# VITA-Group/mm-hand

Hardware: AMD Instinct MI355X
Metric: 256x256 hand images/sec (G+D step) (higher is better)
Workload: dtype f32; 1 GPU; RHD-shaped 256x256, per-GPU batch 32, fp32 (Winograd F(6x6,3x3) on the 3x3 stack), G(9 PATBlocks, ngf64)+D_PB+D_PP+L1/perceptual/GAN+Adam, --norm instance, dropout on; VGG19[:4] weights: random-init (seed 1234): NOT the reference's pretrained objective; global_batch=32, parallelism=dp1

## Files before the change

include/mmhand_hip.h:

```cpp
#ifndef MMHAND_HIP_H
#define MMHAND_HIP_H

#include <stddef.h>
#include <stdint.h>

#ifdef __cplusplus
extern "C" {
#endif
#pragma GCC visibility push(default)

typedef void* mmh_stream_t;

enum { MMH_PAD_ZERO = 0, MMH_PAD_REFLECT = 1 };
enum { MMH_ACT_NONE = 0, MMH_ACT_RELU = 1, MMH_ACT_TANH = 2 };
enum { MMH_F32 = 0, MMH_BF16 = 1, MMH_FP16 = 2 };

typedef struct mmh_conv_desc {
    int32_t B, H, W;
    int32_t Cin, Cout;
    int32_t kh, kw;
    int32_t stride;
    int32_t pad;
    int32_t pad_mode;
    int32_t Ho, Wo;
// ... 150 lines not shown
size_t mmh_colsum_ws_bytes(int64_t rows, int C);
int mmh_colsum(const void* x, int64_t rows, int C, int cs, void* out,
               void* ws, size_t ws_bytes, int accumulate, int x_dtype, mmh_stream_t s);


size_t mmh_norm_stats_ws_bytes(int groups, int64_t rows_per_group, int C);
int mmh_norm_stats(const void* x, int groups, int64_t rows_per_group, int C,
                   int cs, void* mean, void* m2, void* ws, size_t ws_bytes,
                   int x_dtype, mmh_stream_t s);

int mmh_norm_stats_merge(const void* partials, int groups, int chunks, int C, void* mean,
                         void* m2, mmh_stream_t s);

size_t mmh_norm_stats_merge2_ws_bytes(int sub, int C);
int mmh_norm_stats_merge2(const void* partials, int chunks, int C, int sub, void* ws,
                          size_t ws_bytes, void* mean, void* m2, mmh_stream_t s);

int mmh_norm_stats_merge_finalize(const void* partials, int groups, int chunks, int C, double count,
                                  float eps, void* mean, void* m2, void* scale, void* shift,
                                  void* invstd, mmh_stream_t s);
int mmh_syncbn_merge_finalize(const void* gathered, int ranks, int64_t rank_stride, int C, double count,
                              float eps, const void* gamma, const void* beta, void* mean, void* m2,
                              void* scale, void* shift, void* invstd, void* running_mean,
                              void* running_var, float momentum, mmh_stream_t s);
int mmh_norm_finalize(const void* mean, const void* m2, double count,
                      const void* gamma, const void* beta, float eps,
                      int groups, int C, void* scale, void* shift,
                      void* invstd, void* running_mean, void* running_var,
                      float momentum, mmh_stream_t s);

int mmh_scale_shift_act(const void* x, const void* scale, const void* shift,
                        const void* residual, void* out, int groups,
                        int64_t rows_per_group, int C, int relu, float drop_p,
                        uint64_t seed, const void* mask, void* keep_bits,
                        int x_dtype, int out_dtype, mmh_stream_t s);
int mmh_scale_shift_act_twin(const void* x, const void* scale, const void* shift,
                             const void* residual, void* out, int groups,
                             int64_t rows_per_group, int C, int relu, float drop_p,
                             uint64_t seed, const void* mask, void* keep_bits,
                             int x_dtype, int out_dtype, void* twin, int twin_dtype, mmh_stream_t s);

size_t mmh_norm_bwd_ws_bytes(int groups, int64_t rows_per_group, int C);
int mmh_norm_bwd_reduce(const void* g, const void* out, const void* x,
                        const void* mean, const void* invstd, int groups,
                        int64_t rows_per_group, int C, int masked,
                        float drop_p, void* s1, void* s2, void* ws,
                        size_t ws_bytes, int g_dtype, int x_dtype, mmh_stream_t s);
int mmh_norm_bwd_apply(const void* g, const void* out, const void* x,
                       const void* mean, const void* invstd,
                       const void* gamma, const void* s1, const void* s2,
                       double count, int groups, int64_t rows_per_group,
                       int C, int masked, float drop_p, void* dx,
                       int g_dtype, int x_dtype, int dx_dtype, mmh_stream_t s);

int mmh_norm_bwd_fused_supported(int groups, int64_t rows, int C, int masked, int g_dtype, int x_dtype);
int mmh_norm_bwd_fused(const void* g, const void* out, const void* x, const void* mean, const void* invstd,
                       const void* gamma, double count, int groups, int64_t rows, int C, int masked, float drop_p,
                       void* s1, void* s2, void* dx, int g_dtype, int x_dtype, int dx_dtype, mmh_stream_t s);

int mmh_dropout_bits(int64_t n, float drop_p, uint64_t seed, const void* mask, void* bits,
                     mmh_stream_t s);
int mmh_dropout_bits_rows(const void* bits, int64_t image_rows, int W, int C, void* rows,
                          mmh_stream_t s);
int mmh_dropout_bits_both(int64_t image_rows, int W, int C, float drop_p, uint64_t seed,
                          const void* mask, void* bits, void* rows, mmh_stream_t s);
int mmh_norm_bwd_reduce_rc(const void* g, const void* x, const void* mean, const void* invstd,
                           const void* scale, const void* shift, const void* dbits, int groups,
                           int64_t rows_per_group, int C, int relu, float drop_p, void* s1,
                           void* s2, void* ws, size_t ws_bytes, mmh_stream_t s);
int mmh_norm_bwd_apply_rc(const void* g, const void* x, const void* mean, const void* invstd,
                          const void* gamma, const void* s1, const void* s2, const void* scale,
                          const void* shift, const void* dbits, double count, int groups,
                          int64_t rows_per_group, int C, int relu, float drop_p, void* dx,
                          mmh_stream_t s);
int mmh_wino_input_normact(const void* x, int B, int H, int W, int C, int reflect, void* V,
                           const void* scale, const void* shift, int groups, int relu,
                           float drop_p, const void* drows, mmh_stream_t s);
int mmh_wino_input_dy_normbwd(const void* g, const void* x, int B, int H, int W, int C, void* V,
                              void* Yh, int fold, const void* mean, const void* invstd,
                              const void* gamma, const void* s1, const void* s2, double count,
                              const void* scale, const void* shift, const void* drows, int groups,
                              int relu, float drop_p, mmh_stream_t s);

int mmh_act_bwd(const void* g, const void* y, void* dx, int64_t n, int act,
                mmh_stream_t s);
int mmh_act_bwd_lp16(const void* g, const void* y, int64_t n, int act, int dtype, void* out16,
                     mmh_stream_t s);
int mmh_act_bwd_lp16_io(const void* g, int g_is16, const void* y, int y_is16, int64_t n, int act, int dtype,
                        void* out16, mmh_stream_t s);

int mmh_patblock_gate_fwd(const void* x1, const void* s1, const void* s2,
                          const void* s3, void* out, void* x2n, void* x3n,
                          int64_t rows, int C, int cat_dtype, int s23_dtype, mmh_stream_t s);
int mmh_patblock_gate_bwd(const void* g_out, const void* g_x2n,
                          const void* g_x3n, const void* s1, const void* s2,
                          const void* s3, void* g_x1, void* g_s1, void* g_s2,
                          void* g_s3, int64_t rows, int C, int gcat_dtype, int s23_dtype,
                          int gs23_dtype, mmh_stream_t s);

int mmh_patblock_gate_norm_supported(int groups, int64_t rows_per_group, int C);
int mmh_patblock_gate_norm_fwd(const void* x1, const void* y2, const void* scale, const void* shift,
                               const void* s2, const void* s3, void* out, void* x2n, void* x3n, int groups,
                               int64_t rows_per_group, int C, int y_dtype, int cat_dtype, int s23_dtype,
                               mmh_stream_t s);
int mmh_patblock_gate_norm_bwd(const void* g_out, const void* g_x2n, const void* g_x3n, const void* y2,
                               const void* scale, const void* shift, const void* mean, const void* invstd,
                               const void* s2, const void* s3, void* g_x1, void* g_s1, void* g_s2, void* g_s3,
                               void* sum1, void* sum2, void* ws, size_t ws_bytes, int groups,
                               int64_t rows_per_group, int C, int y_dtype, int gcat_dtype, int s23_dtype,
                               mmh_stream_t s);

size_t mmh_reduce_ws_bytes(int64_t n);
int mmh_bce_logits_fwd(const void* x, int64_t n, float target, float weight,
                       double denom, void* out, void* ws, size_t ws_bytes,
                       mmh_stream_t s);
int mmh_bce_logits_bwd(const void* x, int64_t n, float target, float weight,
                       double denom, const void* gscalar, void* dx,
                       mmh_stream_t s);
int mmh_l1_fwd(const void* a, const void* b, int64_t n, float weight,
               double denom, void* out, void* ws, size_t ws_bytes,
               mmh_stream_t s);
int mmh_l1_bwd(const void* a, const void* b, int64_t n, float weight,
               double denom, const void* gscalar, void* da, mmh_stream_t s);
int mmh_l1_fwd_lp16(const void* a16, const void* b16, int64_t n, float weight,
                    double denom, int dtype, void* out, void* ws, size_t ws_bytes,
                    mmh_stream_t s);
int mmh_l1_relu_bwd_lp16(const void* a16, const void* b16, int64_t n, float weight,
                         double denom, const void* gscalar, int dtype, void* out16,
                         mmh_stream_t s);

int mmh_mse_fwd(const void* a, const void* b, int64_t n, float weight,
                double denom, void* out, void* ws, size_t ws_bytes,
                mmh_stream_t s);
int mmh_mse_bwd(const void* a, const void* b, int64_t n, float weight,
                double denom, const void* gscalar, void* da, mmh_stream_t s);

int mmh_maxpool2x2_fwd(const void* x, int B, int H, int W, int C, void* y, mmh_stream_t s);
int mmh_maxpool2x2_bwd(const void* x, const void* g, int B, int H, int W, int C, void* dx, mmh_stream_t s);

int mmh_conv7_thin_fprop(const mmh_conv_desc* d, const void* x, const void* w,
                         const void* bias, void* y, int act, mmh_stream_t s);
size_t mmh_conv7_thin_dgrad_ws_bytes(const mmh_conv_desc* d);
int mmh_conv7_thin_dgrad(const mmh_conv_desc* d, const void* dy, const void* w,
                         void* dx, void* ws, size_t ws_bytes, int dy_dtype, mmh_stream_t s);
size_t mmh_conv7_thin_wgrad_ws_bytes(const mmh_conv_desc* d);
int mmh_conv7_thin_wgrad(const mmh_conv_desc* d, const void* x, const void* dy, void* dw,
                         void* ws, size_t ws_bytes, int accumulate, mmh_stream_t s);

int mmh_conv7_head_dgrad_lp16_supported(const mmh_conv_desc* d);
size_t mmh_conv7_head_dgrad_lp16_ws_bytes(const mmh_conv_desc* d);
int mmh_conv7_head_dgrad_lp16(const mmh_conv_desc* d, const void* dy, const void* w, void* dx, int dx_is16, void* ws,
                              size_t ws_bytes, const void* zeros, mmh_stream_t s);

int mmh_conv7_n4_lp16_supported(const mmh_conv_desc* d, int mode);
size_t mmh_conv7_n4_lp16_ws_bytes(const mmh_conv_desc* d, int mode);
int mmh_conv7_n4_lp16(const mmh_conv_desc* d, int mode, const void* x16, const void* w,
                      const void* bias, void* y, int act, void* ws, size_t ws_bytes,
                      const void* zeros, mmh_stream_t s);

int mmh_conv7_stem_wgrad_supported(const mmh_conv_desc* d);
size_t mmh_conv7_stem_wgrad_ws_bytes(const mmh_conv_desc* d);
int mmh_conv7_stem_wgrad(const mmh_conv_desc* d, const void* x, const void* dy, void* dw,
                         void* ws, size_t ws_bytes, int accumulate, mmh_stream_t s);

int mmh_adam_step(void* p, const void* g, void* m, void* v, int64_t n,
                  float lr, float beta1, float beta2, float eps, int step,
// ... 98 lines not shown
```

mmhand_amd/csrc/common.h:

```cpp
#pragma once
#include <hip/hip_runtime.h>
#include <cstdarg>
#include <cstdio>
#include <cstdint>
#include "../../include/mmhand_hip.h"

namespace mmh {

char* err_buf();
int fail(const char* fmt, ...);

inline int check_launch(const char* what) {
    hipError_t e = hipGetLastError();
    if (e != hipSuccess) return fail("%s: %s", what, hipGetErrorString(e));
    return 0;
}

inline hipStream_t as_stream(mmh_stream_t s) { return reinterpret_cast<hipStream_t>(s); }

inline int64_t cdiv(int64_t a, int64_t b) { return (a + b - 1) / b; }

__device__ __forceinline__ float norm_bwd_elem(float g, bool keep, float dsc, float xv, float mu, float k0, float k1,
                                               float k2) {
    float dz = keep ? g * dsc : 0.f;
// ... 21 lines not shown
        float lo = even[r], hi = odd[r];
        asm volatile("s_nop 1\n\tv_permlane16_swap_b32 %0, %1\n\ts_nop 1" : "+v"(lo), "+v"(hi));
        v[r] = lo;
        v[4 + r] = hi;
    }
}
template <bool H16>
__device__ __forceinline__ void store8_lp16(char* dst, const float* v) {
    if (H16) {
        typedef _Float16 h8 __attribute__((ext_vector_type(8)));
        h8 o;
#pragma unroll
        for (int e = 0; e < 8; ++e) o[e] = (_Float16)v[e];
        *reinterpret_cast<h8*>(dst) = o;
    } else {
        typedef __bf16 b8 __attribute__((ext_vector_type(8)));
        b8 o;
#pragma unroll
        for (int e = 0; e < 8; ++e) o[e] = (__bf16)v[e];
        *reinterpret_cast<b8*>(dst) = o;
    }
}

#define MMH_SWZ_(val, s) __builtin_bit_cast(float, __builtin_amdgcn_ds_swizzle(__builtin_bit_cast(int, val), 0x1f | ((s) << 10)))
template <int NS, int S>
__device__ __forceinline__ void wave_stats_step(float* m, float* q, int& ns, bool bit, float w) {
    if (ns > 1) {
        const int h = ns / 2;
#pragma unroll
        for (int c = 0; c < NS / 2; ++c) {
            if (c < h) {
                const float km = bit ? m[h + c] : m[c], sm = bit ? m[c] : m[h + c];
                const float kq = bit ? q[h + c] : q[c], sq = bit ? q[c] : q[h + c];
                const float om = MMH_SWZ_(sm, S), oq = MMH_SWZ_(sq, S), dl = om - km;
                q[c] = kq + oq + dl * dl * w;
                m[c] = 0.5f * (km + om);
            }
        }
        ns = h;
    } else {
        const float om = MMH_SWZ_(m[0], S), oq = MMH_SWZ_(q[0], S), dl = om - m[0];
        q[0] = q[0] + oq + dl * dl * w;
        m[0] = 0.5f * (m[0] + om);
    }
}
template <int NV, int NJ, typename F>
__device__ __forceinline__ void wave_tile_stats(F val, int l15, float* sp, int N) {
    constexpr int NS = 4 * NJ;
    float m[NS], q[NS];
#pragma unroll
    for (int j = 0; j < NJ; ++j)
#pragma unroll
        for (int r = 0; r < 4; ++r) {
            float v[NV], mean = 0.f, qq = 0.f;
#pragma unroll
            for (int i = 0; i < NV; ++i) { v[i] = val(i, j, r); mean += v[i]; }
            mean *= 1.f / NV;
#pragma unroll
            for (int i = 0; i < NV; ++i) qq = __builtin_fmaf(v[i] - mean, v[i] - mean, qq);
            m[4 * j + r] = mean; q[4 * j + r] = qq;
        }
    int ns = NS;
    wave_stats_step<NS, 8>(m, q, ns, (l15 & 8) != 0, 0.5f * NV);
    wave_stats_step<NS, 4>(m, q, ns, (l15 & 4) != 0, 1.0f * NV);
    wave_stats_step<NS, 2>(m, q, ns, (l15 & 2) != 0, 2.0f * NV);
    wave_stats_step<NS, 1>(m, q, ns, (l15 & 1) != 0, 4.0f * NV);
    constexpr int SPLITS = NS >= 16 ? 4 : (NS >= 8 ? 3 : (NS >= 4 ? 2 : 1));
    const int slot = l15 >> (4 - SPLITS);
    const bool writer = (l15 & ((1 << (4 - SPLITS)) - 1)) == 0;
    if (writer) {
        const int co = (slot >> 2) * 16 + (slot & 3);
        sp[co] = 16.f * NV;
        sp[N + co] = m[0];
        sp[2 * N + co] = q[0];
    }
}

int wino6_weights(const float* w, float* U, int Cin, int Cout, int flip_transpose, hipStream_t st);
int wino6_weights_multi(const long long* table, int n, long long total_blocks, hipStream_t st);
int wino6_input(const float* x, float* V, int B, int H, int W, int C, int reflect, int xcd, hipStream_t st);
int wino6_output(const float* M, float* y, const float* bias, int B, int H, int W, int C, int act, float* stats,
                 int fold, hipStream_t st);
int wino6_dy(const float* dy, float* Yh, int B, int H, int W, int C, hipStream_t st);
int wino6_input_normact(const float* x, float* V, int B, int H, int W, int C, int reflect, int xcd,
                        const float* scale, const float* shift, int groups, int relu, float drop_p,
                        const uint32_t* drows, hipStream_t st);
int wino6_input_dy_normbwd(const float* g, const float* x, float* V, float* Yh, int B, int H, int W, int C, int xcd,
                           int fold, const float* mean, const float* invstd, const float* gamma, const float* s1,
                           const float* s2, double count, const float* scale, const float* shift,
                           const uint32_t* drows, int groups, int relu, float drop_p, hipStream_t st);
int wino6_input_dy(const float* dy, float* V, float* Yh, int B, int H, int W, int C, int xcd, int fold,
                   hipStream_t st);
int wino6_dw(const float* dU, float* dw, int Cin, int Cout, int accumulate, hipStream_t st);
bool wgrad_lp16t_supported(const mmh_conv_desc* d);
int wgrad_lp16t_splits(const mmh_conv_desc* d);
int launch_wgrad_lp16t(const mmh_conv_desc* d, const void* x16, const void* dy16, float* slab, const void* zeros,
                       hipStream_t st);
bool dgrad_s2_halo_ok(const mmh_conv_desc* d, int dx_cs, int act);
int launch_dgrad_s2_halo(const mmh_conv_desc* d, const void* dy, const void* w, const void* bias, void* dx, int dx_cs,
                         int act, hipStream_t st);
extern int g_dgrad_s2_halo, g_dgrad_s2_dbg;
bool wgrad_s2_strip_ok(const mmh_conv_desc* d);
size_t wgrad_s2_strip_ws_bytes(const mmh_conv_desc* d);
int launch_wgrad_s2_strip(const mmh_conv_desc* d, const void* x, const void* dy, void* dw, void* ws, size_t ws_bytes,
                          int accumulate, hipStream_t st);
extern int g_wgrad_s2_strip;
bool stem_f32_ok(const mmh_conv_desc* d);
int stem_f32_stats_chunks(const mmh_conv_desc* d);
int launch_stem_f32(const mmh_conv_desc* d, const void* x, const void* w, const void* bias, void* y, int act, float* stats,
                    hipStream_t st);
extern int g_stem_f32, g_stem_f32_dbg, g_stem_f32_levels;
bool wino_wgrad_dma_ok(int64_t tiles, int Cin, int Cout, int nbatch);
size_t wino_wgrad_dma_ws_bytes(int64_t tiles, int Cin, int Cout, int nbatch);
int launch_wino_wgrad_dma(const float* V, const float* Yh, int64_t tiles, int Cin, int Cout, int nbatch, float* ws, float* dU,
                          hipStream_t st);
extern int g_wino_wgrad_dma;
int launch_slab_reduce(const float* slab, float* dw, int64_t n4_total, int splits, int accumulate, int64_t n4, hipStream_t st);
bool conv_s2f_ok(const mmh_conv_desc* d, int mode);
bool conv_s1f_ok(const mmh_conv_desc* d, int mode);
int conv_s2f_stats_chunks(const mmh_conv_desc* d);
int launch_conv_s2f(const mmh_conv_desc* d, const void* x16, const void* w16, const void* bias, void* y, int y_is16, int act,
                    const void* zeros, hipStream_t st, float* stats = nullptr, int mode = 0);
bool conv_s2d_ok(const mmh_conv_desc* d, int mode);
int launch_conv_s2d(const mmh_conv_desc* d, const void* g16, const void* w16, const void* bias, void* dx, int dx_is16, int act,
                    const void* zeros, hipStream_t st);
extern int g_lp16_s2f;
extern int g_lp16_persist;
extern int g_slab_reduce_par;
extern int g_wino6_vec;
extern int g_lp16_shape;
extern int g_lp16_tap_inner;
extern int g_lp16_dbg;
extern int g_lp16_wgrad_ring;
extern int g_lp16_wgrad_s2;
extern int g_pw_v2;
extern int g_col_chunks, g_row_chunks;

}

#define MMH_REQUIRE(cond, ...)                      \
    do {                                            \
        if (!(cond)) return mmh::fail(__VA_ARGS__); \
    } while (0)
```

mmhand_amd/csrc/conv_igemm.hip:

```cpp
#include <algorithm>
#include <cstring>
#include "common.h"

namespace {

typedef float f32x16 __attribute__((ext_vector_type(16)));
typedef __bf16 bf16x8 __attribute__((ext_vector_type(8)));
typedef __bf16 bf16x4 __attribute__((ext_vector_type(4)));
typedef __bf16 bf16x2 __attribute__((ext_vector_type(2)));
typedef _Float16 f16x8 __attribute__((ext_vector_type(8)));
typedef _Float16 f16x4 __attribute__((ext_vector_type(4)));
typedef _Float16 f16x2 __attribute__((ext_vector_type(2)));
__device__ __forceinline__ bf16x4 to_bf16x4(float4 v) {
    bf16x4 r;
    r[0] = (__bf16)v.x; r[1] = (__bf16)v.y; r[2] = (__bf16)v.z; r[3] = (__bf16)v.w;
    return r;
}
template <bool H16>
__device__ __forceinline__ bf16x4 to_lp4(float4 v) {
    if (H16) {
        f16x4 r;
        r[0] = (_Float16)v.x; r[1] = (_Float16)v.y; r[2] = (_Float16)v.z; r[3] = (_Float16)v.w;
        return __builtin_bit_cast(bf16x4, r);
    }
// ... 2638 lines not shown
            v.x = apply_act(v.x, act); v.y = apply_act(v.y, act);
            yo[(((long long)b * H + 4 * ty + r) * W + 4 * tx + q) * C2 + c] = v;
        }
    }
}

__global__ void wino4_dy_kernel(const float* __restrict__ dy, float* __restrict__ Yh, int B, int H, int W,
                                int C2) {
    const int TH = H / 4, TW = W / 4;
    const long long tiles = (long long)B * TH * TW;
    long long i = (long long)blockIdx.x * blockDim.x + threadIdx.x;
    if (i >= tiles * C2) return;
    const int c = (int)(i % C2);
    const long long tile = i / C2;
    const int tx = (int)(tile % TW), ty = (int)((tile / TW) % TH), b = (int)(tile / ((long long)TW * TH));
    const F2* in = reinterpret_cast<const F2*>(dy);
    F2 yv[4][4], t[6][4], colv[4], o6[6];
#pragma unroll
    for (int r = 0; r < 4; ++r)
#pragma unroll
        for (int q = 0; q < 4; ++q) yv[r][q] = in[(((long long)b * H + 4 * ty + r) * W + 4 * tx + q) * C2 + c];
#pragma unroll
    for (int q = 0; q < 4; ++q) {
#pragma unroll
        for (int r = 0; r < 4; ++r) colv[r] = yv[r][q];
        w4_a(colv, o6);
#pragma unroll
        for (int r = 0; r < 6; ++r) t[r][q] = o6[r];
    }
    const long long plane = tiles * C2;
    F2* out = reinterpret_cast<F2*>(Yh) + tile * C2 + c;
#pragma unroll
    for (int r = 0; r < 6; ++r) {
        w4_a(t[r], o6);
#pragma unroll
        for (int q = 0; q < 6; ++q) out[(long long)(r * 6 + q) * plane] = o6[q];
    }
}

__global__ void wino4_dw_kernel(const float* __restrict__ dU, float* __restrict__ dw, int64_t plane2,
                                int accumulate) {
    int64_t i = (int64_t)blockIdx.x * blockDim.x + threadIdx.x;
    if (i >= plane2) return;
    const F2* in = reinterpret_cast<const F2*>(dU) + i;
    F2 u[6][6], t[3][6], colv[6], o3[3];
#pragma unroll
    for (int a = 0; a < 6; ++a)
#pragma unroll
        for (int b = 0; b < 6; ++b) u[a][b] = in[(int64_t)(a * 6 + b) * plane2];
#pragma unroll
    for (int b = 0; b < 6; ++b) {
#pragma unroll
        for (int a = 0; a < 6; ++a) colv[a] = u[a][b];
        w4_gt(colv, o3);
#pragma unroll
        for (int a = 0; a < 3; ++a) t[a][b] = o3[a];
    }
    F2* out = reinterpret_cast<F2*>(dw) + i;
#pragma unroll
    for (int a = 0; a < 3; ++a) {
        w4_gt(t[a], o3);
#pragma unroll
        for (int b = 0; b < 3; ++b) {
            F2 v = o3[b];
            if (accumulate) v = v + out[(int64_t)(a * 3 + b) * plane2];
            out[(int64_t)(a * 3 + b) * plane2] = v;
        }
    }
}

template <int BN, int WM, int WN, bool NMAJOR>
int launch_batched_t(const BatchKP& bp, int nbatch, hipStream_t st) {
    constexpr size_t lds = (BM * LDA + (NMAJOR ? BN * LDA : BK * BN)) * sizeof(float) + tab_bytes(BM);
    static int ready = -1;
    if (ready != 0) ready = allow_lds(conv_igemm_batched_kernel<BN, WM, WN, NMAJOR>, lds);
    if (ready != 0) return ready;
    dim3 grid((bp.p.N + BN - 1) / BN, (bp.p.M + BM - 1) / BM, nbatch);
    hipLaunchKernelGGL((conv_igemm_batched_kernel<BN, WM, WN, NMAJOR>), grid, dim3(256), lds, st, bp);
    return mmh::check_launch("conv_igemm_batched_kernel");
}

int g_wino_bn256 = 0;
int g_wino_xcd = 1;
int g_wino_gemm_v2 = 1;
int g_wino_bf16_bk = 64;
int g_wino_bf16_occ = 3;
int g_wino_gemm_occ = 3;
int g_wino_gemm_levels = 2;
int g_wino_gemm_bn = 0;

template <int BN, int LEVELS>
static int launch_wino_gemm_t(const WinoGemmKP& p, hipStream_t st) {
    constexpr size_t lds = (size_t)(BM * LDA + BK * BN) * sizeof(float);
    static int ready = -1;
    if (ready != 0) ready = allow_lds(wino_gemm_kernel<BN, LEVELS>, lds);
    if (ready != 0) return ready;
    hipLaunchKernelGGL((wino_gemm_kernel<BN, LEVELS>), dim3(8 * p.nb), dim3(256), lds, st, p);
    return mmh::check_launch("wino_gemm_kernel");
}

static int wino_gemm_v2(const float* V, const float* U, float* Mo, long long tiles, int K, int N, hipStream_t st,
                        int nbatch, int levels, bool fold16 = false) {
    WinoGemmKP p{};
    p.A = V; p.B = U; p.C = Mo;
    p.M = (int)tiles; p.K = K; p.N = N; p.P = nbatch;
    const int bn = g_wino_gemm_bn == 64 ? 64 : (N > 64 ? 128 : 64);
    p.MT = (p.M + BM - 1) / BM;
    p.NT = (N + bn - 1) / bn;
    p.W = nbatch * p.MT * p.NT;
    p.Wx = (p.W + 7) / 8;
    const bool two = (levels ? levels : g_wino_gemm_levels) == 2 && (nbatch == 64 || fold16) && K > WINO_FOLD * BK;
    p.nb = std::min(p.Wx, 32 * g_wino_gemm_occ);
    if (two) return bn == 128 ? launch_wino_gemm_t<128, 2>(p, st) : launch_wino_gemm_t<64, 2>(p, st);
    return bn == 128 ? launch_wino_gemm_t<128, 1>(p, st) : launch_wino_gemm_t<64, 1>(p, st);
}

int wino_gemm(const float* V, const float* U, float* Mo, long long tiles, int K, int N, hipStream_t st,
              int nbatch = 16, int levels = 0) {
    MMH_REQUIRE(tiles * (long long)std::max(K, N) < (1ll << 30), "winograd: tensor too large");
    if (g_wino_gemm_v2 && K % BK == 0 && N >= 64 && N % 32 == 0) return wino_gemm_v2(V, U, Mo, tiles, K, N, st, nbatch, levels);
    BatchKP bp{};
    ConvKP& p = bp.p;
    Gather& g = p.g;
    g.src = V;
    g.src_bytes = (unsigned)((size_t)tiles * K * sizeof(float));
    g.srcH = 1; g.srcW = (int)tiles; g.src_cs = (unsigned)K;
    g.PH = 1; g.PW = (int)tiles; g.TH = 1; g.TW = 1;
    g.C4 = K / 4;
    g.ap_h = 0; g.at_h = 0; g.a0_h = 0; g.ap_w = 1; g.at_w = 0; g.a0_w = 0;
    g.shift = 0; g.reflect = 0;
    set_korder(g, p.nk, p.Kflat);
    p.w = U;
    p.w_bytes = (unsigned)((size_t)K * N * sizeof(float));
    p.out = Mo;
    p.M = (int)tiles; p.N = N;
    p.wCin = K; p.wCout = N;
    p.KW_true = 1; p.kh0 = 0; p.kw0 = 0; p.tstep = 1;
    p.OH = 1; p.OW = (int)tiles; p.o_p = 1;
    p.out_cs = (unsigned)N; p.out_linear = 1;
    p.act = MMH_ACT_NONE;
    bp.src_bs = tiles * K; bp.w_bs = (long long)K * N; bp.out_bs = tiles * N;
    {
        const int bn = (N % 256 == 0 && g_wino_bn256) ? 256 : 128;
        const int gx = (N + bn - 1) / bn, gy = (p.M + BM - 1) / BM;
        p.xcd_remap = (g_conv_xcd && gx > 1 && gy >= 8) ? 1 : 0;
    }
    if (N % 256 == 0 && g_wino_bn256) return launch_batched_t<256, 2, 2, false>(bp, nbatch, st);
    if (N > 64) return launch_batched_t<128, 2, 2, false>(bp, nbatch, st);
    if (N > 32) return launch_batched_t<64, 2, 2, false>(bp, nbatch, st);
    return launch_batched_t<32, 4, 1, false>(bp, nbatch, st);
}

int g_wgrad_slots = 768;
int g_wgrad_bn256 = 1;
int g_wino_wgrad_v2 = 1;
int g_wino_wgrad_occ = 3;
int g_wgrad_xcd = 1;
int g_wino_wgrad_bn256 = 0;
int g_wino_wgrad_slots = 2304;

int wgrad_splits(int Mrows, int N, int P) {
    const int bn = (g_wgrad_bn256 && N % 256 == 0) ? 256 : 128;
    const int tiles = ((Mrows + BM - 1) / BM) * ((N + bn - 1) / bn);
    const int slots = g_wgrad_slots;
    int max_splits = P / (8 * BK);
    if (max_splits > 256) max_splits = 256;
// ... 43 lines not shown

template <int BN, int WM, int WN>
int launch_wgrad_grid_t(const WgradKP& p, dim3 grid, hipStream_t st) {
    constexpr size_t lds = (BK * LDW + BK * BN) * sizeof(float);
    static int ready = -1;
    if (ready != 0) ready = allow_lds(conv_wgrad_kernel<BN, WM, WN, false>, lds);
    if (ready != 0) return ready;
    hipLaunchKernelGGL((conv_wgrad_kernel<BN, WM, WN, false>), grid, dim3(256), lds, st, p);
    return mmh::check_launch("conv_wgrad_kernel");
}

size_t wgrad_ws(const mmh_conv_desc* d) {
    const int Mrows = d->kh * d->kw * d->Cin;
    const int P = d->B * d->Ho * d->Wo;
    const size_t generic = (size_t)wgrad_splits(Mrows, d->Cout, P) * Mrows * d->Cout * sizeof(float);
    return mmh::wgrad_s2_strip_ok(d) ? std::max(generic, mmh::wgrad_s2_strip_ws_bytes(d)) : generic;
}

int do_wgrad(const mmh_conv_desc* d, const void* x, const void* dy, void* dw, void* ws,
             size_t ws_bytes, int accumulate, hipStream_t st, bool x16 = false, bool dy16 = false) {
    MMH_REQUIRE(!(x16 || dy16) || is16(d->dtype), "wgrad: 16-bit operands need a 16-bit dtype");
    MMH_REQUIRE(x16 == dy16, "wgrad: io16 must be 0 (both tensors fp32) or 3 (both 16-bit)");
    if (!x16 && mmh::wgrad_s2_strip_ok(d)) return mmh::launch_wgrad_s2_strip(d, x, dy, dw, ws, ws_bytes, accumulate, st);
    WgradKP p{};
    p.g = fwd_gather(d, x);
    p.g.chunk_major = 0;
    p.x16 = x16 ? 1 : 0;
    p.dy16 = dy16 ? 1 : 0;
    if (x16) p.g.src_bytes /= 2;
    p.dy = static_cast<const float*>(dy);
    p.dy_bytes = (unsigned)((size_t)d->B * d->Ho * d->Wo * d->y_cs * (dy16 ? 2 : sizeof(float)));
    p.dy_cs = (unsigned)d->y_cs;
    p.Mrows = d->kh * d->kw * d->Cin;
    p.N = d->Cout;
    p.P = d->B * d->Ho * d->Wo;
    const int splits = wgrad_splits(p.Mrows, p.N, p.P);
    MMH_REQUIRE(ws_bytes >= (size_t)splits * p.Mrows * p.N * sizeof(float),
                "wgrad workspace too small: %zu < %zu", ws_bytes,
                (size_t)splits * p.Mrows * p.N * sizeof(float));
    p.slab = static_cast<float*>(ws);
    const bool bf16 = is16(d->dtype);
    p.h16 = d->dtype == MMH_FP16;
    p.pix_per_split = (int)(mmh::cdiv(mmh::cdiv(p.P, splits), bf16 ? BKP : BK) * (bf16 ? BKP : BK));
    p.dbg = g_conv_dbg;
    p.nsplit = splits;
    int rc;
    if (bf16) {
        if (p.N > 64) rc = launch_wgrad_bf16_t<128, 2, 2>(p, splits, st);
        else if (p.N > 32) rc = launch_wgrad_bf16_t<64, 2, 2>(p, splits, st);
        else rc = launch_wgrad_bf16_t<32, 4, 1>(p, splits, st);
    } else if (g_wgrad_bn256 && p.N % 256 == 0) rc = launch_wgrad_t<256, 2, 2, false>(p, splits, st);
    else if (p.N > 64) rc = g_wgrad_dbuf ? launch_wgrad_t<128, 2, 2, true>(p, splits, st)
                                    : launch_wgrad_t<128, 2, 2, false>(p, splits, st);
    else if (p.N > 32) rc = launch_wgrad_t<64, 2, 2, false>(p, splits, st);
    else rc = launch_wgrad_t<32, 4, 1, false>(p, splits, st);
    if (rc) return rc;
    const int64_t n4 = (int64_t)p.Mrows * p.N / 4;
    return mmh::launch_slab_reduce(p.slab, static_cast<float*>(dw), n4, splits, accumulate, n4, st);
}

}

extern "C" {

int mmh_set_option(const char* key, int value) {
    MMH_REQUIRE(key != nullptr, "mmh_set_option: NULL key");
    if (!strcmp(key, "conv_dbuf")) { g_conv_dbuf = value; return 0; }
    if (!strcmp(key, "conv_dbg")) { g_conv_dbg = value; return 0; }
    if (!strcmp(key, "conv_cw")) { g_conv_cw = value; return 0; }
    if (!strcmp(key, "conv_bn256")) { g_conv_bn256 = value; return 0; }
    if (!strcmp(key, "conv_levels")) { g_conv_levels = value == 2 ? 2 : 1; mmh::g_stem_f32_levels = g_conv_levels; return 0; }
    if (!strcmp(key, "wino_bn256")) { g_wino_bn256 = value; return 0; }
    if (!strcmp(key, "conv_xcd")) { g_conv_xcd = value; return 0; }
    if (!strcmp(key, "conv_xcd1")) { g_conv_xcd1 = value; return 0; }
    if (!strcmp(key, "conv_tall")) { g_conv_tall = value; return 0; }
    if (!strcmp(key, "wgrad_slots")) { g_wgrad_slots = value; return 0; }
    if (!strcmp(key, "wgrad_dbuf")) { g_wgrad_dbuf = value; return 0; }
    if (!strcmp(key, "wgrad_bn256")) { g_wgrad_bn256 = value; return 0; }
    if (!strcmp(key, "wgrad_xcd")) { g_wgrad_xcd = value; return 0; }
    if (!strcmp(key, "wino_wgrad_v2")) { g_wino_wgrad_v2 = value; return 0; }
    if (!strcmp(key, "wino_wgrad_occ")) { g_wino_wgrad_occ = value; return 0; }
    if (!strcmp(key, "wino_gemm_v2")) { g_wino_gemm_v2 = value; return 0; }
    if (!strcmp(key, "wino_xcd")) { g_wino_xcd = value; return 0; }
    if (!strcmp(key, "dgrad_s2_multi")) { g_dgrad_s2_multi = value; return 0; }
    if (!strcmp(key, "wino6_vec")) { mmh::g_wino6_vec = value; return 0; }
    if (!strcmp(key, "lp16_shape")) { mmh::g_lp16_shape = value; return 0; }
    if (!strcmp(key, "lp16_s2f")) { mmh::g_lp16_s2f = value; return 0; }
    if (!strcmp(key, "lp16_persist")) { mmh::g_lp16_persist = value; return 0; }
    if (!strcmp(key, "lp16_tap_inner")) { mmh::g_lp16_tap_inner = value; return 0; }
    if (!strcmp(key, "pw_v2")) { mmh::g_pw_v2 = value; return 0; }
    if (!strcmp(key, "col_chunks") && value > 0) { mmh::g_col_chunks = value; return 0; }
    if (!strcmp(key, "row_chunks") && value > 0) { mmh::g_row_chunks = value; return 0; }
    if (!strcmp(key, "dgrad_s2_halo")) { mmh::g_dgrad_s2_halo = value; return 0; }
    if (!strcmp(key, "wgrad_s2_strip")) { mmh::g_wgrad_s2_strip = value; return 0; }
    if (!strcmp(key, "stem_f32")) { mmh::g_stem_f32 = value; return 0; }
    if (!strcmp(key, "wino_wgrad_dma")) { mmh::g_wino_wgrad_dma = value; return 0; }
    if (!strcmp(key, "stem_f32_dbg")) { mmh::g_stem_f32_dbg = value; return 0; }
    if (!strcmp(key, "slab_reduce_par")) { mmh::g_slab_reduce_par = value; return 0; }
    if (!strcmp(key, "dgrad_s2_dbg")) { mmh::g_dgrad_s2_dbg = value; return 0; }
    if (!strcmp(key, "lp16_dbg")) { mmh::g_lp16_dbg = value; return 0; }
    if (!strcmp(key, "lp16_wgrad_ring")) { mmh::g_lp16_wgrad_ring = value; return 0; }
    if (!strcmp(key, "lp16_wgrad_s2")) { mmh::g_lp16_wgrad_s2 = value; return 0; }
    if (!strcmp(key, "border_bn64")) { g_border_bn64 = value; return 0; }
    if (!strcmp(key, "wino_gemm_occ")) { g_wino_gemm_occ = value; return 0; }
    if (!strcmp(key, "wino_gemm_levels")) { g_wino_gemm_levels = value; return 0; }
    if (!strcmp(key, "wino_gemm_bn")) { g_wino_gemm_bn = value; return 0; }
    if (!strcmp(key, "wino_bf16_occ")) { g_wino_bf16_occ = value; return 0; }
    if (!strcmp(key, "wino_bf16_bk")) { g_wino_bf16_bk = value; return 0; }
    if (!strcmp(key, "wino_wgrad_bn256")) { g_wino_wgrad_bn256 = value; return 0; }
    if (!strcmp(key, "wino_wgrad_slots")) { g_wino_wgrad_slots = value; return 0; }
    return mmh::fail("mmh_set_option: unknown key '%s'", key);
}

int mmh_conv2d_fprop(const mmh_conv_desc* d, const void* x, const void* w, const void* bias,
                     void* y, int act, mmh_stream_t s) {
    if (int rc = validate(d)) return rc;
    MMH_REQUIRE(x && w && y, "mmh_conv2d_fprop: NULL buffer");
    return do_fprop(d, x, w, bias, y, act, mmh::as_stream(s));
}

int mmh_conv2d_fprop_stats_chunks(const mmh_conv_desc* d) { return d ? fprop_stats_chunks(d) : 0; }

int mmh_conv2d_fprop_stats(const mmh_conv_desc* d, const void* x, const void* w, const void* bias, void* y,
                           void* stats, mmh_stream_t s) {
    if (int rc = validate(d)) return rc;
    MMH_REQUIRE(x && w && y && stats, "mmh_conv2d_fprop_stats: NULL buffer");
    MMH_REQUIRE(fprop_stats_chunks(d) > 0, "mmh_conv2d_fprop_stats: needs fp32 and B*Ho*Wo %% 128 == 0");
    return do_fprop(d, x, w, bias, y, MMH_ACT_NONE, mmh::as_stream(s), static_cast<float*>(stats));
}

int mmh_conv2d_dgrad(const mmh_conv_desc* d, const void* dy, const void* w, void* dx, int dx_cs,
                     mmh_stream_t s) {
    if (int rc = validate(d)) return rc;
    MMH_REQUIRE(dy && w && dx, "mmh_conv2d_dgrad: NULL buffer");
    MMH_REQUIRE(dx_cs % 4 == 0 && dx_cs >= d->Cin, "mmh_conv2d_dgrad: bad dx_cs=%d", dx_cs);
    return do_dgrad(d, dy, w, nullptr, dx, dx_cs, MMH_ACT_NONE, mmh::as_stream(s));
}

static int wino_planes(int tile) { return (tile + 2) * (tile + 2); }
static bool wino_tile_ok(int tile) { return tile == 2 || tile == 4 || tile == 6; }
static bool wino_hw_ok(int H, int W, int tile) {
    return tile == 6 ? (H >= 4 && W >= 4) : (H >= tile + 2 && W >= tile + 2 && H % tile == 0 && W % tile == 0);
}
static long long wino_tiles(int B, int H, int W, int tile) {
    return (long long)B * ((H + tile - 1) / tile) * ((W + tile - 1) / tile);
}

static bool wino_dtype_ok(int dtype, int tile) { return dtype == MMH_F32 || (is16(dtype) && tile == 2); }

int mmh_wino_weights(const void* w, int Cin, int Cout, int flip_transpose, int tile, int dtype, void* U,
                     mmh_stream_t s) {
    MMH_REQUIRE(w && U && Cin > 0 && Cout > 0 && wino_tile_ok(tile) && wino_dtype_ok(dtype, tile),
                "mmh_wino_weights: bad arguments (tile 2 | 4 | 6; bf16 needs tile 2)");
    const dim3 grid((Cin * Cout + 255) / 256);
    if (tile == 6)
        return mmh::wino6_weights(static_cast<const float*>(w), static_cast<float*>(U), Cin, Cout, flip_transpose,
                                  mmh::as_stream(s));
    if (tile == 4)
        hipLaunchKernelGGL(wino4_weights_kernel, grid, dim3(256), 0, mmh::as_stream(s),
                           static_cast<const float*>(w), static_cast<float*>(U), Cin, Cout, flip_transpose);
    else if (dtype == MMH_FP16)
        hipLaunchKernelGGL(wino_weights_kernel<2>, grid, dim3(256), 0, mmh::as_stream(s),
                           static_cast<const float*>(w), U, Cin, Cout, flip_transpose);
    else if (dtype == MMH_BF16)
        hipLaunchKernelGGL(wino_weights_kernel<1>, grid, dim3(256), 0, mmh::as_stream(s),
                           static_cast<const float*>(w), U, Cin, Cout, flip_transpose);
// ... 122 lines not shown
    p.h16 = h16;
    p.MT = (p.M + BM - 1) / BM;
    p.NT = (N + 127) / 128;
    p.W = nbatch * p.MT * p.NT;
    p.Wx = (p.W + 7) / 8;
    if (g_wino_bf16_bk == 128 && K % 128 == 0) {
        p.nb = std::min(p.Wx, 32 * 2);
        constexpr size_t lds = (size_t)(2 * BM * (128 + 8)) * sizeof(__bf16);
        static int ready = -1;
        if (ready != 0) ready = allow_lds(wino_gemm_bf16_kernel<128, false>, lds) | allow_lds(wino_gemm_bf16_kernel<128, true>, lds);
        if (ready != 0) return ready;
        if (h16) hipLaunchKernelGGL((wino_gemm_bf16_kernel<128, true>), dim3(8 * p.nb), dim3(256), lds, st, p);
        else hipLaunchKernelGGL((wino_gemm_bf16_kernel<128, false>), dim3(8 * p.nb), dim3(256), lds, st, p);
    } else {
        p.nb = std::min(p.Wx, 32 * g_wino_bf16_occ);
        constexpr size_t lds = (size_t)(2 * BM * (64 + 8)) * sizeof(__bf16);
        static int ready = -1;
        if (ready != 0) ready = allow_lds(wino_gemm_bf16_kernel<64, false>, lds) | allow_lds(wino_gemm_bf16_kernel<64, true>, lds);
        if (ready != 0) return ready;
        if (h16) hipLaunchKernelGGL((wino_gemm_bf16_kernel<64, true>), dim3(8 * p.nb), dim3(256), lds, st, p);
        else hipLaunchKernelGGL((wino_gemm_bf16_kernel<64, false>), dim3(8 * p.nb), dim3(256), lds, st, p);
    }
    return mmh::check_launch("wino_gemm_bf16_kernel");
}

int mmh_wino_gemm(const void* V, const void* U, void* M, int64_t tiles, int K, int N, int nbatch, int dtype,
                  mmh_stream_t s) {
    MMH_REQUIRE(V && U && M && tiles > 0 && K % 32 == 0 && N % 4 == 0 && nbatch > 0 &&
                    (dtype == MMH_F32 || is16(dtype)),
                "mmh_wino_gemm: bad arguments");
    if (is16(dtype)) return wino_gemm_bf16(V, U, M, tiles, K, N, nbatch, dtype == MMH_FP16, mmh::as_stream(s));
    return wino_gemm(static_cast<const float*>(V), static_cast<const float*>(U), static_cast<float*>(M), tiles,
                     K, N, mmh::as_stream(s), nbatch);
}

int mmh_wino_gemm_levels(const void* V, const void* U, void* M, int64_t tiles, int K, int N, int nbatch, int levels,
                         mmh_stream_t s) {
    MMH_REQUIRE(V && U && M && tiles > 0 && K % 32 == 0 && N % 4 == 0 && nbatch > 0 && (levels == 1 || levels == 2),
                "mmh_wino_gemm_levels: bad arguments (fp32; levels 1 | 2)");
    return wino_gemm(static_cast<const float*>(V), static_cast<const float*>(U), static_cast<float*>(M), tiles, K, N,
                     mmh::as_stream(s), nbatch, levels);
}

int mmh_wino_gemm_levels16(const void* V, const void* U, void* M, int64_t tiles, int K, int N, int levels, mmh_stream_t s) {
    MMH_REQUIRE(V && U && M && tiles > 0 && K > 0 && K % 32 == 0 && N >= 64 && N % 32 == 0 && (levels == 1 || levels == 2),
                "mmh_wino_gemm_levels16: bad arguments (fp32, 16 planes; K %% 32 == 0, N %% 32 == 0, N >= 64; levels 1 | 2)");
    MMH_REQUIRE(tiles * (long long)std::max(K, N) < (1ll << 30), "mmh_wino_gemm_levels16: tensor too large");
    MMH_REQUIRE(g_wino_gemm_v2, "mmh_wino_gemm_levels16: needs the persistent kernel (option wino_gemm_v2)");
    return wino_gemm_v2(static_cast<const float*>(V), static_cast<const float*>(U), static_cast<float*>(M), tiles, K, N,
                        mmh::as_stream(s), 16, levels, true);
}

int mmh_wino_output(const void* M, void* y, const void* bias, int B, int H, int W, int C, int act, int tile,
                    int dtype, void* stats, int fold, mmh_stream_t s) {
    MMH_REQUIRE(M && y && B > 0 && wino_tile_ok(tile) && wino_hw_ok(H, W, tile) && C % 4 == 0 &&
                    wino_dtype_ok(dtype, tile),
                "mmh_wino_output: bad arguments");
    const long long tiles = wino_tiles(B, H, W, tile);
    MMH_REQUIRE(!stats || (tile == 6 && dtype == MMH_F32), "mmh_wino_output: statistics need tile 6, fp32");
    MMH_REQUIRE(!fold || (tile == 6 && dtype == MMH_F32 && wino_fold_ok(H, W) && !bias && !stats && act == MMH_ACT_NONE),
                "mmh_wino_output: fold needs tile 6, fp32, no bias / activation / statistics, (H+1) %% 6 >= 2");
    if (tile == 6)
        return mmh::wino6_output(static_cast<const float*>(M), static_cast<float*>(y), static_cast<const float*>(bias),
                                 B, H, W, C, act, static_cast<float*>(stats), fold ? 1 : 0, mmh::as_stream(s));
    if (tile == 4) {
        const long long total = tiles * (C / 2);
        hipLaunchKernelGGL(wino4_output_kernel, dim3((unsigned)((total + 255) / 256)), dim3(256), 0,
                           mmh::as_stream(s), static_cast<const float*>(M), static_cast<float*>(y),
                           static_cast<const float*>(bias), B, H, W, C / 2, act);
    } else {
        const long long total = tiles * (C / 4);
        const dim3 grid((unsigned)((total + 255) / 256));
        if (dtype == MMH_FP16)
            hipLaunchKernelGGL(wino_output_kernel<2>, grid, dim3(256), 0, mmh::as_stream(s), M,
                               static_cast<float*>(y), static_cast<const float*>(bias), B, H, W, C / 4, act);
        else if (dtype == MMH_BF16)
            hipLaunchKernelGGL(wino_output_kernel<1>, grid, dim3(256), 0, mmh::as_stream(s), M,
                               static_cast<float*>(y), static_cast<const float*>(bias), B, H, W, C / 4, act);
        else
            hipLaunchKernelGGL(wino_output_kernel<0>, grid, dim3(256), 0, mmh::as_stream(s), M,
                               static_cast<float*>(y), static_cast<const float*>(bias), B, H, W, C / 4, act);
    }
    return mmh::check_launch("wino_output_kernel");
}

static int wino_wgrad_splits(int Cin, int Cout, long long tiles, int nbatch) {
    const int bn = (g_wino_wgrad_bn256 && Cout % 256 == 0) ? 256 : 128;
    const int per = ((Cin + BM - 1) / BM) * ((Cout + bn - 1) / bn) * nbatch;
    const int s = std::max(1, g_wino_wgrad_slots / per);
    const long long maxs = std::max<long long>(1, tiles / (8 * BK));
    return (int)std::min<long long>(s, maxs);
}

size_t mmh_wino_wgrad_gemm_ws_bytes(int64_t tiles, int Cin, int Cout, int nbatch) {
    if (tiles <= 0 || Cin <= 0 || Cout <= 0 || nbatch <= 0) return 0;
    const size_t generic = (size_t)nbatch * wino_wgrad_splits(Cin, Cout, tiles, nbatch) * Cin * Cout * sizeof(float);
    return mmh::wino_wgrad_dma_ok(tiles, Cin, Cout, nbatch) ? std::max(generic, mmh::wino_wgrad_dma_ws_bytes(tiles, Cin, Cout, nbatch))
                                                            : generic;
}

int mmh_wino_wgrad_gemm(const void* V, const void* Yh, int64_t tiles, int Cin, int Cout, int nbatch, int dtype,
                        void* ws, size_t ws_bytes, void* dU, mmh_stream_t s) {
    MMH_REQUIRE(V && Yh && ws && dU && tiles > 0 && Cin % 4 == 0 && Cout % 4 == 0 &&
                    (dtype == MMH_F32 || is16(dtype)),
                "mmh_wino_wgrad_gemm: bad arguments");
    MMH_REQUIRE(ws_bytes >= mmh_wino_wgrad_gemm_ws_bytes(tiles, Cin, Cout, nbatch),
                "mmh_wino_wgrad_gemm: workspace too small");
    MMH_REQUIRE(tiles * (long long)std::max(Cin, Cout) < (1ll << 30), "mmh_wino_wgrad_gemm: tensor too large");
    hipStream_t st = mmh::as_stream(s);
    if (dtype == MMH_F32 && mmh::wino_wgrad_dma_ok(tiles, Cin, Cout, nbatch))
        return mmh::launch_wino_wgrad_dma(static_cast<const float*>(V), static_cast<const float*>(Yh), tiles, Cin, Cout, nbatch,
                                          static_cast<float*>(ws), static_cast<float*>(dU), st);
    const int splits = wino_wgrad_splits(Cin, Cout, tiles, nbatch);
    if (is16(dtype)) {
        MMH_REQUIRE(Cin % BM == 0 && Cout % 128 == 0, "mmh_wino_wgrad_gemm (bf16): needs Cin, Cout %% 128 == 0");
        WinoWgradBfKP q{};
        q.h16 = dtype == MMH_FP16;
        q.V = static_cast<const __bf16*>(V); q.Y = static_cast<const __bf16*>(Yh); q.slab = static_cast<float*>(ws);
        q.T = (int)tiles; q.Cin = Cin; q.Cout = Cout; q.P = nbatch;
        q.t_per_split = (int)(mmh::cdiv(mmh::cdiv(tiles, splits), BKP) * BKP);
        q.S = (int)mmh::cdiv(tiles, q.t_per_split);
        q.MT = Cin / BM; q.NT = Cout / 128;
        q.W = nbatch * q.S * q.MT * q.NT;
        q.Wx = (q.W + 7) / 8;
        q.nb = std::min(q.Wx, 32 * g_wino_bf16_occ);
        constexpr size_t lds = (size_t)(2 * BKP * LDT) * sizeof(__bf16);
        static int ready = -1;
        if (ready != 0) ready = allow_lds(wino_wgrad_gemm_bf16_kernel<false>, lds) | allow_lds(wino_wgrad_gemm_bf16_kernel<true>, lds);
        if (ready != 0) return ready;
        if (q.h16) hipLaunchKernelGGL(wino_wgrad_gemm_bf16_kernel<true>, dim3(8 * q.nb), dim3(256), lds, st, q);
        else hipLaunchKernelGGL(wino_wgrad_gemm_bf16_kernel<false>, dim3(8 * q.nb), dim3(256), lds, st, q);
        if (int rc = mmh::check_launch("wino_wgrad_gemm_bf16_kernel")) return rc;
        const int64_t n4 = (int64_t)Cin * Cout / 4;
        return mmh::launch_slab_reduce(q.slab, static_cast<float*>(dU), nbatch * n4, q.S, 0, n4, st);
    }
    if (g_wino_wgrad_v2 && Cin % BM == 0 && Cout % 128 == 0) {
        WinoWgradKP q{};
        q.V = static_cast<const float*>(V); q.Y = static_cast<const float*>(Yh); q.slab = static_cast<float*>(ws);
        q.T = (int)tiles; q.Cin = Cin; q.Cout = Cout; q.P = nbatch;
        q.t_per_split = (int)(mmh::cdiv(mmh::cdiv(tiles, splits), BK) * BK);
        q.S = (int)mmh::cdiv(tiles, q.t_per_split);
        q.MT = Cin / BM; q.NT = Cout / 128;
        q.W = nbatch * q.S * q.MT * q.NT;
        q.Wx = (q.W + 7) / 8;
        const int occ = g_wino_wgrad_occ == 4 ? 4 : 3;
        q.nb = std::min(q.Wx, 32 * occ);
        constexpr size_t lds = (size_t)(BK * LDW + BK * 128) * sizeof(float);
        static int ready3 = -1, ready4 = -1;
        if (occ == 4) {
            if (ready4 != 0) ready4 = allow_lds(wino_wgrad_gemm_kernel<4>, lds);
            if (ready4 != 0) return ready4;
            hipLaunchKernelGGL(wino_wgrad_gemm_kernel<4>, dim3(8 * q.nb), dim3(256), lds, st, q);
        } else {
            if (ready3 != 0) ready3 = allow_lds(wino_wgrad_gemm_kernel<3>, lds);
            if (ready3 != 0) return ready3;
            hipLaunchKernelGGL(wino_wgrad_gemm_kernel<3>, dim3(8 * q.nb), dim3(256), lds, st, q);
        }
        if (int rc = mmh::check_launch("wino_wgrad_gemm_kernel")) return rc;
        const int64_t n4 = (int64_t)Cin * Cout / 4;
        return mmh::launch_slab_reduce(q.slab, static_cast<float*>(dU), nbatch * n4, q.S, 0, n4, st);
    }
    WgradKP p{};
    Gather& g = p.g;
    g.src = static_cast<const float*>(V);
    g.src_bytes = (unsigned)((size_t)tiles * Cin * sizeof(float));
    g.srcH = 1; g.srcW = (int)tiles; g.src_cs = (unsigned)Cin;
// ... 126 lines not shown
```

mmhand_amd/csrc/wino6.hip:

```cpp
#include "common.h"

namespace {

struct F2 { float x, y; };
__device__ __forceinline__ F2 operator+(F2 a, F2 b) { return {a.x + b.x, a.y + b.y}; }
__device__ __forceinline__ F2 operator-(F2 a, F2 b) { return {a.x - b.x, a.y - b.y}; }
__device__ __forceinline__ F2 operator*(float k, F2 a) { return {k * a.x, k * a.y}; }

__device__ __forceinline__ float act6(float v, int act) {
    if (act == MMH_ACT_RELU) return v > 0.f ? v : 0.f;
    if (act == MMH_ACT_TANH) return tanhf(v);
    return v;
}

template <typename T>
__device__ __forceinline__ void w6_bt(const T* d, T* o) {
    const T e1 = d[2] - 4.25f * d[4] + d[6], f1 = d[1] - 4.25f * d[3] + d[5];
    const T e2 = 0.25f * d[2] - 1.25f * d[4] + d[6], f2 = 0.5f * d[1] - 2.5f * d[3] + 2.f * d[5];
    const T e3 = 4.f * d[2] - 5.f * d[4] + d[6], f3 = 2.f * d[1] - 2.5f * d[3] + 0.5f * d[5];
    o[0] = d[0] - d[6] + 5.25f * (d[4] - d[2]);
    o[1] = e1 + f1; o[2] = e1 - f1;
    o[3] = e2 + f2; o[4] = e2 - f2;
    o[5] = e3 + f3; o[6] = e3 - f3;
    o[7] = d[7] - d[1] + 5.25f * (d[3] - d[5]);
// ... 262 lines not shown
    const long long tiles = (long long)B * TH * TW;
    const long long i = (long long)blockIdx.x * blockDim.x + threadIdx.x;
    if (i >= tiles * C2) return;
    const int c = (int)(i % C2);
    const long long tile = i / C2;
    const int tx = (int)(tile % TW), ty = (int)((tile / TW) % TH), b = (int)(tile / ((long long)TW * TH));
    const long long plane = tiles * C2;
    const T* in = reinterpret_cast<const T*>(M) + tile * C2 + c;
    T s6[6][8], colv[8], o6[6];
#pragma unroll
    for (int q = 0; q < 8; ++q) {
#pragma unroll
        for (int r = 0; r < 8; ++r) colv[r] = in[(long long)(r * 8 + q) * plane];
        w6_at(colv, o6);
#pragma unroll
        for (int r = 0; r < 6; ++r) s6[r][q] = o6[r];
    }
    const T bv = bias ? reinterpret_cast<const T*>(bias)[c] : zero_of(T{});
    T* yo = reinterpret_cast<T*>(y);
    T vals[6][6];
    if (fold) {
#pragma unroll
        for (int r = 0; r < 6; ++r) {
            w6_at(s6[r], o6);
#pragma unroll
            for (int q = 0; q < 6; ++q) vals[r][q] = o6[q];
        }
        const int rb = H + 1 - 6 * ty, cb = W + 1 - 6 * tx;
#pragma unroll
        for (int q = 0; q < 6; ++q) {
            if (ty == 0) vals[2][q] = vals[2][q] + vals[0][q];
#pragma unroll
            for (int r = 2; r < 6; ++r)
                if (r == rb) vals[r - 2][q] = vals[r - 2][q] + vals[r][q];
        }
#pragma unroll
        for (int r = 0; r < 6; ++r) {
            if (tx == 0) vals[r][2] = vals[r][2] + vals[r][0];
#pragma unroll
            for (int q = 2; q < 6; ++q)
                if (q == cb) vals[r][q - 2] = vals[r][q - 2] + vals[r][q];
        }
#pragma unroll
        for (int r = 0; r < 6; ++r) {
            const int ph = 6 * ty + r;
#pragma unroll
            for (int q = 0; q < 6; ++q) {
                const int pw = 6 * tx + q;
                if (ph >= 1 && ph <= H && pw >= 1 && pw <= W)
                    yo[(((long long)b * H + ph - 1) * W + pw - 1) * C2 + c] = vals[r][q];
            }
        }
        return;
    }
    float n = 0.f, sum = 0.f;
#pragma unroll
    for (int r = 0; r < 6; ++r) {
        const int hh = 6 * ty + r;
        w6_at(s6[r], o6);
#pragma unroll
        for (int q = 0; q < 6; ++q) {
            const int ww = 6 * tx + q;
            vals[r][q] = act_of(o6[q] + bv, act);
            if (hh < H && ww < W) {
                yo[(((long long)b * H + hh) * W + ww) * C2 + c] = vals[r][q];
                stat_add(vals[r][q], n, sum);
            }
        }
    }
    if (stats && sizeof(T) == 4) {
        const float mean = sum / n;
        float m2 = 0.f;
#pragma unroll
        for (int r = 0; r < 6; ++r)
#pragma unroll
            for (int q = 0; q < 6; ++q)
                if (6 * ty + r < H && 6 * tx + q < W) {
                    const float d = *reinterpret_cast<const float*>(&vals[r][q]) - mean;
                    m2 += d * d;
                }
        float* o = stats + ((long long)(b * (TH * TW) + ty * TW + tx) * 3) * C2 + c;
        o[0] = n; o[C2] = mean; o[2 * C2] = m2;
    }
}

template <typename T>
__global__ void __launch_bounds__(256) wino6_dy_kernel(const float* __restrict__ dy, float* __restrict__ Yh, int B,
                                                       int H, int W, int C2) {
    const int TH = (H + 5) / 6, TW = (W + 5) / 6;
    const long long tiles = (long long)B * TH * TW;
    const long long i = (long long)blockIdx.x * blockDim.x + threadIdx.x;
    if (i >= tiles * C2) return;
    const int c = (int)(i % C2);
    const long long tile = i / C2;
    const int tx = (int)(tile % TW), ty = (int)((tile / TW) % TH), b = (int)(tile / ((long long)TW * TH));
    const T* in = reinterpret_cast<const T*>(dy);
    T t[8][6], colv[6], o8[8];
#pragma unroll
    for (int q = 0; q < 6; ++q) {
        const int ww = 6 * tx + q;
#pragma unroll
        for (int r = 0; r < 6; ++r) {
            const int hh = 6 * ty + r;
            colv[r] = (hh < H && ww < W) ? in[(((long long)b * H + hh) * W + ww) * C2 + c] : zero_of(T{});
        }
        w6_a(colv, o8);
#pragma unroll
        for (int r = 0; r < 8; ++r) t[r][q] = o8[r];
    }
    const long long plane = tiles * C2;
    T* out = reinterpret_cast<T*>(Yh) + tile * C2 + c;
#pragma unroll
    for (int r = 0; r < 8; ++r) {
        w6_a(t[r], o8);
#pragma unroll
        for (int q = 0; q < 8; ++q) out[(long long)(r * 8 + q) * plane] = o8[q];
    }
}

template <typename T>
__device__ __forceinline__ void dy_transforms(T (&d)[8][8], float* __restrict__ V, float* __restrict__ Yh,
                                              long long plane, long long at, int fold) {
    T colv[8], o8[8];
    {
        T t[8][6];
#pragma unroll
        for (int q = 0; q < 6; ++q) {
#pragma unroll
            for (int r = 0; r < 6; ++r) colv[r] = fold ? d[r + 2][q + 2] : d[r + 1][q + 1];
            w6_a(colv, o8);
#pragma unroll
            for (int r = 0; r < 8; ++r) t[r][q] = o8[r];
        }
        T* out = reinterpret_cast<T*>(Yh) + at;
#pragma unroll
        for (int r = 0; r < 8; ++r) {
            w6_a(t[r], o8);
#pragma unroll
            for (int q = 0; q < 8; ++q) out[(long long)(r * 8 + q) * plane] = o8[q];
        }
    }
#pragma unroll
    for (int q = 0; q < 8; ++q) {
#pragma unroll
        for (int r = 0; r < 8; ++r) colv[r] = d[r][q];
        w6_bt(colv, o8);
#pragma unroll
        for (int r = 0; r < 8; ++r) d[r][q] = o8[r];
    }
    T* out = reinterpret_cast<T*>(V) + at;
#pragma unroll
    for (int r = 0; r < 8; ++r) {
        w6_bt(d[r], o8);
#pragma unroll
        for (int q = 0; q < 8; ++q) out[(long long)(r * 8 + q) * plane] = o8[q];
    }
}

template <typename T>
__global__ void __launch_bounds__(256) wino6_input_dy_kernel(const float* __restrict__ dy, float* __restrict__ V,
                                                             float* __restrict__ Yh, int B, int H, int W, int C2,
                                                             int xcd_remap, int fold) {
    const int org = fold ? 2 : 1;
    const int TH = (H + 5) / 6, TW = (W + 5) / 6;
    const long long tiles = (long long)B * TH * TW;
    unsigned blk = blockIdx.x;
// ... 87 lines not shown
                const int rr = 2 * stage + r;
                bool keep = !nb.relu || __builtin_fmaf(xw[r][q], sc, sf) > 0.f;
                if (DROP) {
                    const uint32_t wsel = (wg.ww[q] >> 5) == wq0 ? lo[r] : hi[r];
                    keep = keep && ((wsel >> (wg.ww[q] & 31)) & 1u);
                }
                const float o = mmh::norm_bwd_elem(d[rr][q], keep, nb.np.dsc, xw[r][q], mu, k0, k1, k2);
                d[rr][q] = (wg.okh[rr] && wg.okw[q]) ? o : 0.f;
            }
        __builtin_amdgcn_sched_barrier(0);
    }
    dy_transforms(d, V, Yh, tiles * C, tile * C + c, fold);
}

__global__ void __launch_bounds__(256) wino6_dw_kernel(const float* __restrict__ dU, float* __restrict__ dw, int64_t plane2, int accumulate) {
    const int64_t i = (int64_t)blockIdx.x * blockDim.x + threadIdx.x;
    if (i >= plane2) return;
    const F2* in = reinterpret_cast<const F2*>(dU) + i;
    F2 t[3][8], colv[8], o3[3];
#pragma unroll
    for (int q = 0; q < 8; ++q) {
#pragma unroll
        for (int r = 0; r < 8; ++r) colv[r] = in[(int64_t)(r * 8 + q) * plane2];
        w6_gt(colv, o3);
#pragma unroll
        for (int r = 0; r < 3; ++r) t[r][q] = o3[r];
    }
    F2* out = reinterpret_cast<F2*>(dw) + i;
#pragma unroll
    for (int a = 0; a < 3; ++a) {
        w6_gt(t[a], o3);
#pragma unroll
        for (int b = 0; b < 3; ++b) {
            F2 v = o3[b];
            if (accumulate) v = v + out[(int64_t)(a * 3 + b) * plane2];
            out[(int64_t)(a * 3 + b) * plane2] = v;
        }
    }
}

}

namespace mmh {

int wino6_weights(const float* w, float* U, int Cin, int Cout, int flip_transpose, hipStream_t st) {
    hipLaunchKernelGGL(wino6_weights_kernel, dim3((Cin * Cout + 255) / 256), dim3(256), 0, st, w, U, Cin, Cout,
                       flip_transpose);
    return check_launch("wino6_weights_kernel");
}

int wino6_weights_multi(const long long* table, int n, long long total_blocks, hipStream_t st) {
    hipLaunchKernelGGL(wino6_weights_multi_kernel, dim3((unsigned)total_blocks), dim3(256), 0, st, table, n);
    return check_launch("wino6_weights_multi_kernel");
}

int g_wino6_vec = 0x0;

int wino6_input(const float* x, float* V, int B, int H, int W, int C, int reflect, int xcd, hipStream_t st) {
    const int ext = reflect == 2 ? 7 : 5;
    const long long tiles = (long long)B * ((H + ext) / 6) * ((W + ext) / 6);
    const int cpt = (g_wino6_vec & 1) ? 2 : 1;
    const unsigned nblk = (unsigned)((tiles * (C / cpt) + 255) / 256);
    const int remap = (xcd && nblk % 8 == 0 && nblk >= 64) ? 1 : 0;
    if (cpt == 2)
        hipLaunchKernelGGL(wino6_input_kernel<F2>, dim3(nblk), dim3(256), 0, st, x, V, B, H, W, C / 2, reflect, remap);
    else
        hipLaunchKernelGGL(wino6_input_kernel<float>, dim3(nblk), dim3(256), 0, st, x, V, B, H, W, C, reflect, remap);
    return check_launch("wino6_input_kernel");
}

int wino6_output(const float* M, float* y, const float* bias, int B, int H, int W, int C, int act, float* stats,
                 int fold, hipStream_t st) {
    const int ext = fold ? 7 : 5;
    const long long tiles = (long long)B * ((H + ext) / 6) * ((W + ext) / 6);
    if ((g_wino6_vec & 2) && !stats)
        hipLaunchKernelGGL(wino6_output_kernel<F2>, dim3((unsigned)((tiles * (C / 2) + 255) / 256)), dim3(256), 0, st, M,
                           y, bias, B, H, W, C / 2, act, nullptr, fold);
    else
        hipLaunchKernelGGL(wino6_output_kernel<float>, dim3((unsigned)((tiles * C + 255) / 256)), dim3(256), 0, st, M, y,
                           bias, B, H, W, C, act, stats, fold);
    return check_launch("wino6_output_kernel");
}

int wino6_dy(const float* dy, float* Yh, int B, int H, int W, int C, hipStream_t st) {
    const long long tiles = (long long)B * ((H + 5) / 6) * ((W + 5) / 6);
    if (g_wino6_vec & 4)
        hipLaunchKernelGGL(wino6_dy_kernel<F2>, dim3((unsigned)((tiles * (C / 2) + 255) / 256)), dim3(256), 0, st, dy, Yh,
                           B, H, W, C / 2);
    else
        hipLaunchKernelGGL(wino6_dy_kernel<float>, dim3((unsigned)((tiles * C + 255) / 256)), dim3(256), 0, st, dy, Yh, B,
                           H, W, C);
    return check_launch("wino6_dy_kernel");
}

int wino6_input_normact(const float* x, float* V, int B, int H, int W, int C, int reflect, int xcd,
                        const float* scale, const float* shift, int groups, int relu, float drop_p,
                        const uint32_t* drows, hipStream_t st) {
    const long long tiles = (long long)B * ((H + 5) / 6) * ((W + 5) / 6);
    const unsigned nblk = (unsigned)((tiles * C + 255) / 256);
    const int remap = (xcd && nblk % 8 == 0 && nblk >= 64) ? 1 : 0;
    NormPro np{scale, shift, drows, (W + 31) / 32, groups == 1 ? 0 : 1, relu ? 0.f : -INFINITY, 1.f / (1.f - drop_p)};
    if (drows)
        hipLaunchKernelGGL(wino6_input_normact_kernel<true>, dim3(nblk), dim3(256), 0, st, x, V, B, H, W, C, reflect,
                           remap, np);
    else
        hipLaunchKernelGGL(wino6_input_normact_kernel<false>, dim3(nblk), dim3(256), 0, st, x, V, B, H, W, C, reflect,
                           remap, np);
    return check_launch("wino6_input_normact_kernel");
}

int wino6_input_dy_normbwd(const float* g, const float* x, float* V, float* Yh, int B, int H, int W, int C, int xcd,
                           int fold, const float* mean, const float* invstd, const float* gamma, const float* s1,
                           const float* s2, double count, const float* scale, const float* shift,
                           const uint32_t* drows, int groups, int relu, float drop_p, hipStream_t st) {
    const long long tiles = (long long)B * ((H + 5) / 6) * ((W + 5) / 6);
    const unsigned nblk = (unsigned)((tiles * C + 255) / 256);
    const int remap = (xcd && nblk % 8 == 0 && nblk >= 64) ? 1 : 0;
    NormBwdPro nb{x, mean, invstd, gamma, s1, s2, (float)(1.0 / count), relu,
                  NormPro{scale, shift, drows, (W + 31) / 32, groups == 1 ? 0 : 1, 0.f, 1.f / (1.f - drop_p)}};
    if (drows)
        hipLaunchKernelGGL(wino6_input_dy_normbwd_kernel<true>, dim3(nblk), dim3(256), 0, st, g, V, Yh, B, H, W, C, remap,
                           fold, nb);
    else
        hipLaunchKernelGGL(wino6_input_dy_normbwd_kernel<false>, dim3(nblk), dim3(256), 0, st, g, V, Yh, B, H, W, C, remap,
                           fold, nb);
    return check_launch("wino6_input_dy_normbwd_kernel");
}

int wino6_input_dy(const float* dy, float* V, float* Yh, int B, int H, int W, int C, int xcd, int fold,
                   hipStream_t st) {
    const long long tiles = (long long)B * ((H + 5) / 6) * ((W + 5) / 6);
    const unsigned nblk = (unsigned)((tiles * C + 255) / 256);
    hipLaunchKernelGGL(wino6_input_dy_kernel<float>, dim3(nblk), dim3(256), 0, st, dy, V, Yh, B, H, W, C,
                       (xcd && nblk % 8 == 0 && nblk >= 64) ? 1 : 0, fold);
    return check_launch("wino6_input_dy_kernel");
}

int wino6_dw(const float* dU, float* dw, int Cin, int Cout, int accumulate, hipStream_t st) {
    const int64_t n2 = (int64_t)Cin * Cout / 2;
    hipLaunchKernelGGL(wino6_dw_kernel, dim3((unsigned)cdiv(n2, 256)), dim3(256), 0, st, dU, dw, n2, accumulate);
    return check_launch("wino6_dw_kernel");
}

}
```

mmhand_amd/lib.py:

```python
import ctypes as C
import os

_HERE = os.path.dirname(os.path.abspath(__file__))
LIB_PATH = os.environ.get("MMH_LIB_PATH") or os.path.join(_HERE, "libmmhand_hip.so")

PAD_ZERO, PAD_REFLECT = 0, 1
ACT_NONE, ACT_RELU, ACT_TANH = 0, 1, 2
F32, BF16, FP16 = 0, 1, 2
U8 = 3


class ConvDesc(C.Structure):
    _fields_ = [(n, C.c_int32) for n in (
        "B", "H", "W", "Cin", "Cout", "kh", "kw", "stride", "pad", "pad_mode",
        "Ho", "Wo", "x_cs", "y_cs", "dtype")]


class PlaneSrc(C.Structure):
    _fields_ = [("ptr", C.c_void_p), ("C", C.c_int32),
                ("sb", C.c_int64), ("sc", C.c_int64), ("sh", C.c_int64), ("sw", C.c_int64)]


class ImageSrc(C.Structure):
    _fields_ = [("ptr", C.c_void_p), ("dtype", C.c_int32), ("scale", C.c_float), ("offset", C.c_float),
# ... 42 lines not shown
    "mmh_conv7_thin_dgrad_ws_bytes": (_sz, [_DP]),
    "mmh_conv7_thin_dgrad": (_i, [_DP, _vp, _vp, _vp, _vp, _sz, _i, _vp]),
    "mmh_conv7_thin_wgrad_ws_bytes": (_sz, [_DP]),
    "mmh_conv7_thin_wgrad": (_i, [_DP, _vp, _vp, _vp, _vp, _sz, _i, _vp]),
    "mmh_conv7_stem_wgrad_supported": (_i, [_DP]),
    "mmh_conv7_stem_wgrad_ws_bytes": (_sz, [_DP]),
    "mmh_conv7_stem_wgrad": (_i, [_DP, _vp, _vp, _vp, _vp, _sz, _i, _vp]),
    "mmh_conv2d_wgrad_ws_bytes": (_sz, [_DP]),
    "mmh_conv2d_wgrad": (_i, [_DP, _vp, _vp, _vp, _vp, _sz, _i, _i, _vp]),
    "mmh_convT2d_fprop": (_i, [_DP, _vp, _vp, _vp, _vp, _i, _i, _vp]),
    "mmh_convT2d_dgrad": (_i, [_DP, _vp, _vp, _vp, _vp]),
    "mmh_convT2d_wgrad": (_i, [_DP, _vp, _vp, _vp, _vp, _sz, _i, _i, _vp]),
    "mmh_reflect_fold": (_i, [_vp, _vp, _i, _i, _i, _i, _i, _vp]),
    "mmh_prep_weights_bf16": (_i, [_vp, _i, _i, _i, _vp, _vp, _vp]),
    "mmh_prep_weights_bf16_flat": (_i, [_vp, _i, _i, _i, _vp, _vp]),
    "mmh_prep_weights_fp16": (_i, [_vp, _i, _i, _i, _vp, _vp, _vp]),
    "mmh_prep_weights_fp16_flat": (_i, [_vp, _i, _i, _i, _vp, _vp]),
    "mmh_cvt_lp16": (_i, [_vp, _i64, _i, _vp, _vp]),
    "mmh_conv_lp16_supported": (_i, [_DP, _i]),
    "mmh_conv_lp16": (_i, [_DP, _i, _vp, _vp, _vp, _vp, _i, _i, _vp, _vp]),
    "mmh_conv_lp16_stats_chunks": (_i, [_DP]),
    "mmh_conv_lp16_fprop_stats": (_i, [_DP, _vp, _vp, _vp, _vp, _vp, _vp, _vp]),
    "mmh_conv_stem16_stats_chunks": (_i, [_DP, _i]),
    "mmh_conv_stem16_stats": (_i, [_DP, _vp, _i, _vp, _vp, _vp, _vp, _vp, _vp]),
    "mmh_lp16_pad_cvt": (_i, [_vp, _i64, _i, _i, _i, _vp, _vp]),
    "mmh_prep_weights_lp16_flat8": (_i, [_vp, _i, _i, _i, _i, _i, _vp, _vp]),
    "mmh_conv_lp16_flat_supported": (_i, [_DP, _i]),
    "mmh_conv_lp16_flat": (_i, [_DP, _vp, _i, _vp, _vp, _vp, _i, _i, _vp, _vp]),
    "mmh_conv_stem16_supported": (_i, [_DP, _i]),
    "mmh_dgrad_s2_halo_supported": (_i, [_DP, _i]),
    "mmh_conv_stem16_weights_bytes": (_sz, [_i]),
    "mmh_prep_weights_stem16": (_i, [_vp, _i, _i, _i, _vp, _vp]),
    "mmh_conv_stem16_weights_bytes_k": (_sz, [_i, _i]),
    "mmh_prep_weights_stem16_k": (_i, [_vp, _i, _i, _i, _i, _vp, _vp]),
    "mmh_conv_stem16": (_i, [_DP, _vp, _i, _vp, _vp, _vp, _i, _i, _vp, _vp]),
    "mmh_wgrad_stem_lp16_supported": (_i, [_DP, _i]),
    "mmh_wgrad_stem_lp16_ws_bytes": (_sz, [_DP, _i]),
    "mmh_wgrad_stem_lp16": (_i, [_DP, _vp, _i, _vp, _vp, _vp, _sz, _i, _vp, _vp]),
    "mmh_conv7_head_wgrad_lp16_supported": (_i, [_DP]),
    "mmh_conv7_head_wgrad_lp16_ws_bytes": (_sz, [_DP]),
    "mmh_conv7_head_wgrad_lp16": (_i, [_DP, _vp, _vp, _vp, _vp, _sz, _i, _vp, _vp]),
    "mmh_wgrad_lp16_flat_supported": (_i, [_DP, _i]),
    "mmh_wgrad_lp16_flat_ws_bytes": (_sz, [_DP, _i]),
    "mmh_wgrad_lp16_flat": (_i, [_DP, _vp, _i, _i, _vp, _vp, _vp, _sz, _i, _vp, _vp]),
    "mmh_conv7_head_dgrad_lp16_supported": (_i, [_DP]),
    "mmh_conv7_head_dgrad_lp16_ws_bytes": (_sz, [_DP]),
    "mmh_conv7_head_dgrad_lp16": (_i, [_DP, _vp, _vp, _vp, _i, _vp, _sz, _vp, _vp]),
    "mmh_conv7_n4_lp16_supported": (_i, [_DP, _i]),
    "mmh_conv7_n4_lp16_ws_bytes": (_sz, [_DP, _i]),
    "mmh_conv7_n4_lp16": (_i, [_DP, _i, _vp, _vp, _vp, _vp, _i, _vp, _sz, _vp, _vp]),
    "mmh_conv3x3_lp16_supported": (_i, [_DP]),
    "mmh_conv3x3_lp16_fold_supported": (_i, [_DP]),
    "mmh_wgrad3x3_lp16_ws_bytes": (_sz, [_DP]),
    "mmh_wgrad3x3_lp16": (_i, [_DP, _vp, _vp, _vp, _vp, _sz, _i, _vp, _vp]),
    "mmh_conv3x3_lp16": (_i, [_DP, _i, _vp, _vp, _vp, _vp, _i, _i, _vp, _vp]),
    "mmh_conv3x3_lp16_stats_chunks": (_i, [_DP]),
    "mmh_conv3x3_lp16_dgrad_nbr_chunks": (_i, [_DP, _i]),
    "mmh_conv3x3_lp16_dgrad_nbr": (_i, [_DP, _i, _vp, _vp, _vp, _vp, _vp, _vp, _vp, _i, _f, _vp, _vp, _vp, _sz, _vp, _vp]),
    "mmh_norm_bwd_sums_final": (_i, [_vp, _i, _i, _i, _vp, _vp, _vp]),
    "mmh_conv3x3_lp16_dgrad_add_supported": (_i, [_DP]),
    "mmh_conv3x3_lp16_dgrad_add": (_i, [_DP, _i, _vp, _vp, _vp, _vp, _vp, _vp]),
    "mmh_conv3x3_lp16_fprop_stats": (_i, [_DP, _vp, _vp, _vp, _vp, _vp, _vp, _vp]),
    "mmh_colsum_ws_bytes": (_sz, [_i64, _i]),
    "mmh_colsum": (_i, [_vp, _i64, _i, _i, _vp, _vp, _sz, _i, _i, _vp]),
    "mmh_norm_stats_ws_bytes": (_sz, [_i, _i64, _i]),
    "mmh_norm_stats": (_i, [_vp, _i, _i64, _i, _i, _vp, _vp, _vp, _sz, _i, _vp]),
    "mmh_norm_finalize": (_i, [_vp, _vp, _d, _vp, _vp, _f, _i, _i, _vp, _vp, _vp, _vp, _vp, _f, _vp]),
    "mmh_syncbn_merge_finalize": (_i, [_vp, _i, _i64, _i, _d, _f, _vp, _vp, _vp, _vp, _vp, _vp, _vp, _vp, _vp, _f, _vp]),
    "mmh_scale_shift_act": (_i, [_vp, _vp, _vp, _vp, _vp, _i, _i64, _i, _i, _f, _u64, _vp, _vp, _i, _i, _vp]),
    "mmh_scale_shift_act_twin": (_i, [_vp, _vp, _vp, _vp, _vp, _i, _i64, _i, _i, _f, _u64, _vp, _vp, _i, _i, _vp, _i, _vp]),
    "mmh_norm_bwd_ws_bytes": (_sz, [_i, _i64, _i]),
    "mmh_norm_bwd_reduce": (_i, [_vp, _vp, _vp, _vp, _vp, _i, _i64, _i, _i, _f, _vp, _vp, _vp, _sz, _i, _i, _vp]),
    "mmh_norm_bwd_apply": (_i, [_vp, _vp, _vp, _vp, _vp, _vp, _vp, _vp, _d, _i, _i64, _i, _i, _f, _vp, _i, _i, _i, _vp]),
    "mmh_norm_bwd_fused_supported": (_i, [_i, _i64, _i, _i, _i, _i]),
    "mmh_norm_bwd_fused": (_i, [_vp, _vp, _vp, _vp, _vp, _vp, _d, _i, _i64, _i, _i, _f, _vp, _vp, _vp, _i, _i, _i, _vp]),
    "mmh_dropout_bits": (_i, [_i64, _f, _u64, _vp, _vp, _vp]),
    "mmh_dropout_bits_rows": (_i, [_vp, _i64, _i, _i, _vp, _vp]),
    "mmh_dropout_bits_both": (_i, [_i64, _i, _i, _f, _u64, _vp, _vp, _vp, _vp]),
    "mmh_norm_bwd_reduce_rc": (_i, [_vp, _vp, _vp, _vp, _vp, _vp, _vp, _i, _i64, _i, _i, _f, _vp, _vp, _vp, _sz, _vp]),
    "mmh_norm_bwd_apply_rc": (_i, [_vp, _vp, _vp, _vp, _vp, _vp, _vp, _vp, _vp, _vp, _d, _i, _i64, _i, _i, _f, _vp, _vp]),
    "mmh_wino_input_normact": (_i, [_vp, _i, _i, _i, _i, _i, _vp, _vp, _vp, _i, _i, _f, _vp, _vp]),
    "mmh_wino_input_dy_normbwd": (_i, [_vp, _vp, _i, _i, _i, _i, _vp, _vp, _i, _vp, _vp, _vp, _vp, _vp, _d, _vp, _vp,
                                       _vp, _i, _i, _f, _vp]),
    "mmh_act_bwd": (_i, [_vp, _vp, _vp, _i64, _i, _vp]),
    "mmh_act_bwd_lp16": (_i, [_vp, _vp, _i64, _i, _i, _vp, _vp]),
    "mmh_act_bwd_lp16_io": (_i, [_vp, _i, _vp, _i, _i64, _i, _i, _vp, _vp]),
    "mmh_patblock_gate_fwd": (_i, [_vp, _vp, _vp, _vp, _vp, _vp, _vp, _i64, _i, _i, _i, _vp]),
    "mmh_patblock_gate_bwd": (_i, [_vp, _vp, _vp, _vp, _vp, _vp, _vp, _vp, _vp, _vp, _i64, _i, _i, _i, _i, _vp]),
    "mmh_patblock_gate_norm_supported": (_i, [_i, _i64, _i]),
    "mmh_patblock_gate_norm_fwd": (_i, [_vp, _vp, _vp, _vp, _vp, _vp, _vp, _vp, _vp, _i, _i64, _i, _i, _i, _i, _vp]),
    "mmh_patblock_gate_norm_bwd": (_i, [_vp, _vp, _vp, _vp, _vp, _vp, _vp, _vp, _vp, _vp, _vp, _vp, _vp, _vp, _vp, _vp, _vp, _sz,
                                        _i, _i64, _i, _i, _i, _i, _vp]),
    "mmh_reduce_ws_bytes": (_sz, [_i64]),
    "mmh_bce_logits_fwd": (_i, [_vp, _i64, _f, _f, _d, _vp, _vp, _sz, _vp]),
    "mmh_bce_logits_bwd": (_i, [_vp, _i64, _f, _f, _d, _vp, _vp, _vp]),
    "mmh_l1_fwd": (_i, [_vp, _vp, _i64, _f, _d, _vp, _vp, _sz, _vp]),
    "mmh_l1_bwd": (_i, [_vp, _vp, _i64, _f, _d, _vp, _vp, _vp]),
    "mmh_l1_fwd_lp16": (_i, [_vp, _vp, _i64, _f, _d, _i, _vp, _vp, _sz, _vp]),
    "mmh_l1_relu_bwd_lp16": (_i, [_vp, _vp, _i64, _f, _d, _vp, _i, _vp, _vp]),
    "mmh_mse_fwd": (_i, [_vp, _vp, _i64, _f, _d, _vp, _vp, _sz, _vp]),
    "mmh_maxpool2x2_fwd": (_i, [_vp, _i, _i, _i, _i, _vp, _vp]),
    "mmh_maxpool2x2_bwd": (_i, [_vp, _vp, _i, _i, _i, _i, _vp, _vp]),
    "mmh_mse_bwd": (_i, [_vp, _vp, _i64, _f, _d, _vp, _vp, _vp]),
    "mmh_adam_step": (_i, [_vp, _vp, _vp, _vp, _i64, _f, _f, _f, _f, _i, _f, _vp, _vp, _vp]),
    "mmh_grad_nonfinite": (_i, [_vp, _i64, _vp, _vp, _vp, _vp]),
    "mmh_loss_scale_update": (_i, [_vp, _vp, _f, _f, _i, _f, _f, _vp]),
    "mmh_pack_nhwc": (_i, [C.POINTER(PlaneSrc), _i, _vp, _i, _i, _i, _i, _i, _vp]),
    "mmh_pack_nhwc_lp16": (_i, [C.POINTER(PlaneSrc), _i, _vp, _vp, _i, _i, _i, _i, _i, _i, _vp]),
    "mmh_pose_heatmaps": (_i, [_vp, _i, _i, _i, _d, _vp, _vp]),
    "mmh_map_to_cord": (_i, [_vp, _i, _i, _i, _f, _vp, _vp]),
    "mmh_decode_inputs": (_i, [_vp, _vp, _vp, _vp, _vp, _vp, _i, _i, _i, _d, _vp, _vp, _vp, _vp, _vp]),
    "mmh_decode_inputs_resized": (_i, [_vp, _vp, _vp, _vp, _vp, _vp, _i, _i, _i, _i, _i, _d, _vp, _vp, _vp, _vp, _vp]),
    "mmh_rccl_bind": (_i, [C.c_char_p]),
    "mmh_rccl_comm_ranks": (_i, [_vp]),
    "mmh_allreduce_bucket": (_i, [_vp, _vp, _i64, _i, _vp]),
    "mmh_image_metrics_ws_bytes": (_sz, [_i, _i, _i, _i, _i]),
    "mmh_image_metrics": (_i, [C.POINTER(ImageSrc), C.POINTER(ImageSrc), _i, _i, _i, _i, _i, _vp, _d, _d, _vp, _sz, _vp, _vp]),
    "mmh_png_decode_batch": (_i, [_vp, _i64, _vp, _i, _i, _i, _vp, _vp, _vp, _i, _vp]),
    "mmh_png_encode_slot_bytes": (_i64, [_i, _i]),
    "mmh_png_encode_scratch_bytes": (_i64, [_i, _i, _i]),
    "mmh_png_encode_batch": (_i, [_vp, _i, _i, _i, _i, _vp, _vp, _i64, _vp, _vp, _vp]),
}

_lib = None


def load():
    global _lib
    if _lib is not None:
        return _lib
    if not os.path.exists(LIB_PATH):
        raise RuntimeError(
            f"{LIB_PATH} not found: build it with `python -c 'import __graft_entry__ as g; g.build()'` "
            "or `make -C mmhand_amd/csrc`.  There is no CPU fallback for the HIP path.")
    lib = C.CDLL(LIB_PATH)
    for name, (res, args) in SIGNATURES.items():
        fn = getattr(lib, name)
        fn.restype = res
        fn.argtypes = args
    _lib = lib
    for item in filter(None, (x.strip() for x in os.environ.get("MMH_OPTIONS", "").split(","))):
        key, sep, val = item.partition("=")
        try:
            ival = int(val)
        except ValueError:
            ival = None
        if not sep or ival is None:
            raise RuntimeError(f"MMH_OPTIONS: '{item}' is not key=integer")
        check(lib.mmh_set_option(key.strip().encode(), ival), f"MMH_OPTIONS {item}")
    return lib


def check(rc, what):
    if rc != 0:
        msg = load().mmh_last_error()
        raise RuntimeError(f"{what} failed: {msg.decode() if msg else 'unknown error'}")


def call(name, *args):
    rc = getattr(_lib or load(), name)(*args)
    if rc != 0:
        check(rc, name)
```

mmhand_amd/networks.py:

```python
import functools
import math

import torch
import torch.nn as nn

from . import lib as L
from . import ops
from .ops import pad4


class ConvParam(nn.Module):

    def __init__(self, cin, cout, k, bias, transposed=False):
        super().__init__()
        self.cin, self.cout, self.k, self.transposed = cin, cout, k, transposed
        a, b = (pad4(cout), pad4(cin)) if transposed else (pad4(cin), pad4(cout))
        self.weight = nn.Parameter(torch.zeros(k, k, a, b))
        self.bias = nn.Parameter(torch.zeros(pad4(cout))) if bias else None

    def logical_weight(self):
        w = self.weight.detach()
        if self.transposed:
            return w.permute(3, 2, 0, 1)[: self.cin, : self.cout]
        return w.permute(3, 2, 0, 1)[: self.cout, : self.cin]
# ... 218 lines not shown
                    q, r = torch.linalg.qr(flat.t() if shape[0] < fan_in else flat)
                    q = q * torch.sign(torch.diagonal(r)).unsqueeze(0)
                    w = (q.t() if shape[0] < fan_in else q).reshape(shape)
                b = None
                if m.bias is not None:
                    bound = 1.0 / math.sqrt((m.cout if m.transposed else m.cin) * rf)
                    b = (torch.rand(m.cout, generator=g) * 2 - 1) * bound
                m.set_logical(w, b)
            elif isinstance(m, NormParam):
                with torch.no_grad():
                    m.weight.copy_(1.0 + torch.randn(m.weight.shape, generator=g) * 0.02)
                    m.bias.zero_()
        return self

    def conv(self, cp, x, stride=1, pad=0, reflect=False, act=L.ACT_NONE, dx_channels=0, y_lp=False, to_norm=False,
             g_defer=False, res_tok=None, x_twin=None):
        x16 = None
        if isinstance(x, tuple):
            x, x16 = x
        if isinstance(x16, ops.NormDefer):
            return ops.Conv2dFn.apply(x, cp.weight, cp.bias, stride, pad, reflect, act, self.bf16, dx_channels, None,
                                      False, bool(to_norm and self.norm == "instance" and self.training), x16, g_defer)
        nb = bool(to_norm and self.training and (self.norm == "instance" or cp.bias is None))
        if x16 is not None:
            res_tok = None
        if y_lp:
            p, y16 = ops.Conv2dFn.apply(x, cp.weight, cp.bias, stride, pad, reflect, act, self.bf16, dx_channels, x16, True, nb,
                                        None, False, res_tok, x_twin)
            return p, y16
        return ops.Conv2dFn.apply(x, cp.weight, cp.bias, stride, pad, reflect, act, self.bf16, dx_channels, x16, False, nb,
                                  None, g_defer, res_tok, x_twin)

    def _lp_edge(self, cp, stride=1, reflect=True):
        if not (self.bf16 and self.training and cp is not None and cp.k == 3):
            return 0
        ws = cp.weight.shape
        if cp.transposed:
            return self.bf16 if ops.convT_lp16_ok(ws[3], ws[2], self.bf16) else 0
        return self.bf16 if ops.lp16_chain_ok(ws[2], ws[3], 3, stride, 1, reflect, self.bf16) else 0

    def _lp_edge_head(self, cp, x):
        if not (self.bf16 and self.training and ops.USE_LP16_EDGES and cp is not None and cp.k == 7):
            return 0
        B, H, W, _ = (x[0] if isinstance(x, tuple) else x).shape
        ws = cp.weight.shape
        return self.bf16 if ops.head16_ok(B, H, W, ws[2], ws[3], 7, 1, 3, True, self.bf16) else 0

    def _lp_out(self, cp, stride=1, reflect=True):
        return bool(ops.USE_LP16_EDGES and self._lp_edge(cp, stride, reflect))

    def _lp_out_stem(self, cp, B, H, W, input_grad, dx_channels=0):
        if not (self.bf16 and self.training and ops.USE_LP16_EDGES) or (input_grad and not 0 < dx_channels <= 4):
            return False
        ws = cp.weight.shape
        d = ops.conv_desc(B, H, W, ws[2], ws[3], cp.k, 1, cp.k // 2, True)
        return ops.stem_lp16_ok(d, self.bf16, dx_channels)

    def convT(self, cp, x, y_lp=False, to_norm=False):
        x16 = None
        if isinstance(x, tuple):
            x, x16 = x
        nb = bool(to_norm and self.norm == "instance" and self.training)
        if y_lp:
            p, y16 = ops.ConvT2dFn.apply(x, cp.weight, cp.bias, self.bf16, x16, True, nb)
            return p, y16
        return ops.ConvT2dFn.apply(x, cp.weight, cp.bias, self.bf16, x16, False, nb)

    def normact(self, bag, idx, x, relu, drop=False, site=None, residual=None, out_lp=0, defer=0, res_tok=None, want_twin=0):
        x16 = None
        if isinstance(x, tuple):
            x, x16 = x
        drop_p = 0.5 if (drop and self.training) else 0.0
        mask = None
        seed = 0
        if drop_p > 0:
            if self._mask_src is not None:
                mask = self._mask_src[site]
            else:
                seed = ops.next_dropout_seed()
        if defer == 3:
            assert self.training and x16 is None and not out_lp and not relu and not drop
            if self.norm == "instance":
                return ops.NormActFn.apply(x, None, None, residual, None, None, "instance", False, 0.0, 0, None, None,
                                           0, None, 3)
            np_ = bag[idx]
            np_.count_batch()
            return ops.NormActFn.apply(x, np_.weight, np_.bias, residual, np_.running_mean, np_.running_var, "batch",
                                       False, 0.0, 0, None, self.sync_group, 0, None, 3)
        if defer:
            assert self.training and x16 is None and residual is None and not out_lp
            if self.norm == "instance":
                args, groups = (None, None, None, None, None, "instance"), x.shape[0]
                sync = None
            else:
                np_ = bag[idx]
                np_.count_batch()
                args, groups = (np_.weight, np_.bias, None, np_.running_mean, np_.running_var, "batch"), 1
                sync = self.sync_group
            p, scale, shift, drows = ops.NormActFn.apply(x, *args, relu, drop_p, seed, mask, sync, 0, None, defer)
            return p, ops.NormDefer(x.detach(), scale, shift, groups, relu, drop_p, drows)
        want_twin = want_twin if (self.training and not out_lp) else 0
        if self.norm == "instance":
            return ops.NormActFn.apply(x, None, None, residual, None, None, "instance", relu,
                                       drop_p, seed, mask, None, out_lp, x16, 0, res_tok, want_twin)
        np_ = bag[idx]
        if self.training:
            np_.count_batch()
            return ops.NormActFn.apply(x, np_.weight, np_.bias, residual, np_.running_mean,
                                       np_.running_var, "batch", relu, drop_p, seed, mask,
                                       self.sync_group, out_lp, x16, 0, res_tok, want_twin)
        scale = np_.weight / torch.sqrt(np_.running_var + ops.EPS)
        shift = np_.bias - np_.running_mean * scale
        y = ops.AffineActFn.apply(x, scale, shift, relu)
        return y if residual is None else y + residual

    def _norm_fusion(self, c1, c2, x):
        if not (ops.USE_NORM_FUSION and self.training and not self.bf16 and torch.is_tensor(x)
                and ops.KEEP_WINOGRAD_INPUT):
            return 0
        B, H, W, Cin = x.shape
        C1, C2 = c1.weight.shape[3], c2.weight.shape[3]
        if not (ops.norm_fusion_ok(C1) and B * H * W * C1 < 2 ** 31 and ops._wino_tile(B, H, W, C1, C2, 3, 1, 1, False) == 6):
            return 0
        null_db = c1.bias is None or (self.norm == "instance" and ops.EXACT_NULL_BIAS_GRAD)
        if (null_db and ops.FUSE_WINO6_BWD and ops._wino_tile(B, H, W, Cin, C1, 3, 1, 1, False) == 6
                and ops._wino_tile(B, H, W, Cin, C1, 3, 1, 1, False, "dgrad") == 6):
            return 2
        return 1

    def _norm_bwd_fusion(self, c2, x):
        if not (ops.USE_NORM_FUSION and self.training and not self.bf16 and ops.KEEP_WINOGRAD_INPUT and ops.FUSE_WINO6_BWD):
            return False
        B, H, W, _ = x.shape
        Cin, Cout = c2.weight.shape[2], c2.weight.shape[3]
        null_db = c2.bias is None or (self.norm == "instance" and ops.EXACT_NULL_BIAS_GRAD)
        return (null_db and ops.norm_fusion_ok(Cout) and B * H * W * Cout < 2 ** 31
                and ops._wino_tile(B, H, W, Cin, Cout, 3, 1, 1, False) == 6
                and ops._wino_tile(B, H, W, Cin, Cout, 3, 1, 1, False, "dgrad") == 6)

    def _res_token(self, x):
        return ops.ResidualToken() if (ops.USE_RESIDUAL_TOKENS and self.bf16 and self.training and torch.is_tensor(x)
                                       and x.requires_grad) else None

    def _twin_for(self, cp):
        if not (self.bf16 and self.training and cp is not None and cp.k == 3 and not cp.transposed):
            return 0
        ws = cp.weight.shape
        return self.bf16 if (ops.lp16_v2_ok(ws[2], ws[3], 3, 1, 1, 0) and ops.norm_twin_ok(ws[2])) else 0

    def two_conv_block(self, blk, x, site, last_norm, residual=None, res_tok=None, x_twin=None, want_twin=0):
        if residual is not None and residual is x and last_norm:
            res_tok = self._res_token(x)
        i2 = 6 if self.use_dropout else 5
        fuse = self._norm_fusion(blk[1], blk[i2], x)
        fuse_last = 3 if (last_norm and last_norm != "gate" and torch.is_tensor(x) and self._norm_bwd_fusion(blk[i2], x)) else 0
        y = self.conv(blk[1], x, 1, 1, True, y_lp=self._lp_out(blk[1]), to_norm=True, g_defer=fuse == 2, res_tok=res_tok,
                      x_twin=x_twin if torch.is_tensor(x) else None)
        y = self.normact(blk, 2, y, True, self.use_dropout, site, out_lp=self._lp_edge(blk[i2]), defer=fuse)
        y = self.conv(blk[i2], y, 1, 1, True, y_lp=self._lp_out(blk[i2]), to_norm=bool(last_norm), g_defer=fuse_last == 3)
        if last_norm == "gate":
            return y
        if last_norm:
            y = self.normact(blk, i2 + 1, y, False, residual=residual, defer=fuse_last,
                             res_tok=res_tok if residual is not None else None, want_twin=want_twin if not fuse_last else 0)
        return y


def two_conv_blocks_lockstep(entries):
    pre = []
    for e in entries:
        net, blk, x = e["net"], e["blk"], e["x"]
        i2 = 6 if net.use_dropout else 5
        fuse = net._norm_fusion(blk[1], blk[i2], x)
        fuse_last = 3 if (e["last_norm"] and torch.is_tensor(x) and net._norm_bwd_fusion(blk[i2], x)) else 0
        y = net.conv(blk[1], x, 1, 1, True, y_lp=net._lp_out(blk[1]), to_norm=True, g_defer=fuse == 2)
        pre.append((i2, fuse, fuse_last, y))
    ys = normact_multi([dict(net=e["net"], bag=e["blk"], idx=2, x=y, relu=True, drop=e["net"].use_dropout and e["net"].training,
                             site=e["site"], out_lp=e["net"]._lp_edge(e["blk"][i2]), defer=fuse)
                        for e, (i2, fuse, fuse_last, y) in zip(entries, pre)])
    zs = []
    for e, (i2, fuse, fuse_last, _), y in zip(entries, pre, ys):
        net, blk = e["net"], e["blk"]
        zs.append(net.conv(blk[i2], y, 1, 1, True, y_lp=net._lp_out(blk[i2]), to_norm=e["last_norm"], g_defer=fuse_last == 3))
    last = [i for i, e in enumerate(entries) if e["last_norm"]]
    if last:
        outs = normact_multi([dict(net=entries[i]["net"], bag=entries[i]["blk"], idx=pre[i][0] + 1, x=zs[i], relu=False,
                                   residual=entries[i].get("residual"), defer=pre[i][2]) for i in last])
        for i, o in zip(last, outs):
            zs[i] = o
    return zs


class Generator(_Net):

    def __init__(self, input_nc, output_nc, ngf=64, norm_layer=nn.BatchNorm2d, use_dropout=False,
                 n_blocks=6, gpu_ids=[], padding_type="reflect", n_downsampling=2):
        assert type(input_nc) == list and len(input_nc) == 3, \
            "The AttModule take input_nc in format of list only!!"
        assert n_blocks >= 0
        if padding_type != "reflect":
            raise NotImplementedError("padding [%s] is not implemented" % padding_type)
        super().__init__(norm_layer, use_dropout)
        self.input_nc, self.output_nc, self.ngf = list(input_nc), output_nc, ngf
        self.n_blocks, self.n_down = n_blocks, n_downsampling
        self.gpu_ids = gpu_ids
        m = self.model = Bag()
        for s, nc in zip((1, 2, 3), input_nc):
            d = m.put(f"stream{s}_down", Bag())
            self._conv(d, 1, nc, ngf, 7)
            self._normp(d, 2, ngf)
            for i in range(n_downsampling):
                c = ngf * 2 ** i
                self._conv(d, 4 + 3 * i, c, 2 * c, 3)
                self._normp(d, 5 + 3 * i, 2 * c)
        dim = ngf * 2 ** n_downsampling
        att = m.put("att", Bag())
        i2 = 6 if use_dropout else 5
        for b in range(n_blocks):
            blk = att.put(b, Bag())
            for s in (1, 2, 3):
                cb = blk.put(f"conv_block_stream{s}", Bag())
                wide = (s != 1) and b > 0
                cin = 2 * dim if wide else dim
                self._conv(cb, 1, cin, cin, 3)
                self._normp(cb, 2, cin)
                self._conv(cb, i2, cin, dim, 3)
                if s == 1:
                    self._normp(cb, i2 + 1, dim)
        up = m.put("stream1_up", Bag())
        for i in range(n_downsampling):
            c = ngf * 2 ** (n_downsampling - i)
            self._conv(up, 3 * i, c, c // 2, 3, transposed=True)
            self._normp(up, 3 * i + 1, c // 2)
        self._conv(up, 3 * n_downsampling + 1, ngf, output_nc, 7, bias=True)

    def _down_lockstep(self, x1, x2, x3):
        m = self.model
        ds = [m[f"stream{s}_down"] for s in (1, 2, 3)]
        xs = [x1, x2, x3]
        first = [d[4] if self.n_down > 0 else None for d in ds]
        ys = []
        for d, x in zip(ds, xs):
            Bx, Hx, Wx, _ = x.shape
            ys.append(self.conv(d[1], x, 1, 3, True, y_lp=self._lp_out_stem(d[1], Bx, Hx, Wx, x.requires_grad), to_norm=True))
        xs = normact_multi([dict(net=self, bag=d, idx=2, x=y, relu=True, out_lp=self._lp_edge(f, 2, False))
                            for d, y, f in zip(ds, ys, first)])
        for i in range(self.n_down):
            ys, lps = [], []
            for s, d, x in zip((1, 2, 3), ds, xs):
                cp = d[4 + 3 * i]
                if i + 1 < self.n_down:
                    out_lp = self._lp_edge(d[4 + 3 * (i + 1)], 2, False)
                elif s != 1 and self.n_blocks > 0:
                    out_lp = self._lp_edge(m["att"][0][f"conv_block_stream{s}"][1])
                else:
                    out_lp = 0
                lps.append(out_lp)
                ys.append(self.conv(cp, x, 2, 1, False, y_lp=self._lp_out(cp, 2, False), to_norm=True))
            xs = normact_multi([dict(net=self, bag=d, idx=5 + 3 * i, x=y, relu=True, out_lp=lp)
                                for d, y, lp in zip(ds, ys, lps)])
        return xs

    def forward_nhwc(self, x1, x2, x3):
        m = self.model
        xs = []
        x1_twin0 = None
        if packing(self):
            x1, x2, x3 = self._down_lockstep(x1, x2, x3)
        for s, x in (() if packing(self) else zip((1, 2, 3), (x1, x2, x3))):
            d = m[f"stream{s}_down"]
            first = d[4] if self.n_down > 0 else None
            Bx, Hx, Wx, _ = x.shape
            x = self.normact(d, 2, self.conv(d[1], x, 1, 3, True, y_lp=self._lp_out_stem(d[1], Bx, Hx, Wx, x.requires_grad), to_norm=True),
                             True, out_lp=self._lp_edge(first, 2, False))
            for i in range(self.n_down):
                cp = d[4 + 3 * i]
                if i + 1 < self.n_down:
                    out_lp = self._lp_edge(d[4 + 3 * (i + 1)], 2, False)
                elif s != 1 and self.n_blocks > 0:
                    out_lp = self._lp_edge(m["att"][0][f"conv_block_stream{s}"][1])
                else:
                    out_lp = 0
                wt = (self._twin_for(m["att"][0]["conv_block_stream1"][1])
                      if (s == 1 and i + 1 == self.n_down and self.n_blocks > 0 and not out_lp) else 0)
                x = self.normact(d, 5 + 3 * i, self.conv(cp, x, 2, 1, False, y_lp=self._lp_out(cp, 2, False), to_norm=True), True,
                                 out_lp=out_lp, want_twin=wt)
                if wt:
                    x, x1_twin0 = x
            xs.append(x)
        if not packing(self):
            x1, x2, x3 = xs
        for b in range(self.n_blocks):
            blk = m["att"][b]
            p = f"model.att.{b}.conv_block_stream"
            tok = None
            x1_twin = x2[1][..., x1.shape[3]:] if (b > 0 and isinstance(x2, tuple) and torch.is_tensor(x1)) else None
            if b == 0 and torch.is_tensor(x1):
                x1_twin = x1_twin0
            if packing(self):
                s1, s2, s3 = two_conv_blocks_lockstep(
                    [dict(net=self, blk=blk[f"conv_block_stream{s}"], x=x, site=p + str(s), last_norm=s == 1)
                     for s, x in zip((1, 2, 3), (x1, x2, x3))])
            else:
                tok = self._res_token(x1)
                i2 = 6 if self.use_dropout else 5
                gate_norm = bool(self.norm == "instance" and self.training and self.bf16 and torch.is_tensor(x1)
                                 and self._lp_out(blk["conv_block_stream1"][i2])
                                 and ops.gate_norm_ok(x1.shape[0], x1.shape[1] * x1.shape[2], x1.shape[3]))
                s1 = self.two_conv_block(blk["conv_block_stream1"], x1, p + "1", "gate" if gate_norm else True, res_tok=tok,
                                         x_twin=x1_twin)
                s2 = self.two_conv_block(blk["conv_block_stream2"], x2, p + "2", False)
                s3 = self.two_conv_block(blk["conv_block_stream3"], x3, p + "3", False)
            more = b + 1 < self.n_blocks
            cat_lp = self._lp_edge(m["att"][b + 1]["conv_block_stream2"][1]) if more else 0
            s16 = (None, None)
            if isinstance(s2, tuple):
                (s2, a), (s3, b_) = s2, s3
                s16 = (a, b_)
            gate_norm = isinstance(s1, tuple)
            if cat_lp:
                if gate_norm:
                    x1, p2, p3, c2, c3 = ops.GateNormFn.apply(x1, s1[0], s2, s3, True, cat_lp, s1[1], *s16, tok)
                else:
                    x1, p2, p3, c2, c3 = ops.GateFn.apply(x1, s1, s2, s3, True, cat_lp, *s16, tok)
                x2, x3 = (p2, c2), (p3, c3)
            elif gate_norm:
                x1, x2, x3 = ops.GateNormFn.apply(x1, s1[0], s2, s3, more, 0, s1[1], *s16, tok)
            else:
                x1, x2, x3 = ops.GateFn.apply(x1, s1, s2, s3, more, 0, *s16, tok)
        up = m["stream1_up"]
        y = x1
        for i in range(self.n_down):
            nxt = up[3 * (i + 1)] if i + 1 < self.n_down else None
            yc = self.convT(up[3 * i], y, y_lp=self._lp_out(up[3 * i]), to_norm=True)
            out_lp = self._lp_edge(nxt) if nxt is not None else self._lp_edge_head(up[3 * self.n_down + 1], yc)
            y = self.normact(up, 3 * i + 1, yc, True, out_lp=out_lp)
        return self.conv(up[3 * self.n_down + 1], y, 1, 3, True, L.ACT_TANH)

    def forward(self, input):
        xs = []
        for x, nc in zip(input, self.input_nc):
            B, Cc, H, W = x.shape
            assert Cc == nc
            xs.append(ops.PackFn.apply(pad4(nc), x.float(), True, nc))
        y = self.forward_nhwc(*xs)
        return ops.nhwc_to_nchw_view(y, self.output_nc)


class Discriminator(_Net):

    def __init__(self, input_nc, ngf=64, norm_layer=nn.BatchNorm2d, use_dropout=False, n_blocks=6,
                 gpu_ids=[], padding_type="reflect", use_sigmoid=False, n_downsampling=2):
        assert n_blocks >= 0
        if padding_type != "reflect":
            raise NotImplementedError("padding [%s] is not implemented" % padding_type)
        if use_sigmoid or n_downsampling > 2:
            raise NotImplementedError("use_sigmoid / n_downsampling>2 are not on the MM-HAND path")
        super().__init__(norm_layer, use_dropout)
        self.input_nc, self.ngf, self.n_blocks, self.n_down = input_nc, ngf, n_blocks, n_downsampling
        self.gpu_ids = gpu_ids
        m = self.model = Bag()
        self._conv(m, 1, input_nc, ngf, 7)
        self._normp(m, 2, ngf)
        for i in range(n_downsampling):
            c = ngf * 2 ** i
            self._conv(m, 4 + 3 * i, c, 2 * c, 3)
            self._normp(m, 5 + 3 * i, 2 * c)
        dim = ngf * 2 ** n_downsampling
        i2 = 6 if use_dropout else 5
        base = 4 + 3 * n_downsampling
        for b in range(n_blocks):
            cb = m.put(base + b, Bag()).put("conv_block", Bag())
            self._conv(cb, 1, dim, dim, 3)
            self._normp(cb, 2, dim)
            self._conv(cb, i2, dim, dim, 3)
            self._normp(cb, i2 + 1, dim)

    def forward_nhwc(self, x, dx_channels=0):
        m = self.model
        first = m[4] if self.n_down > 0 else None
        Bx, Hx, Wx, _ = x.shape
        y = self.normact(m, 2, self.conv(m[1], x, 1, 3, True, dx_channels=dx_channels, to_norm=True,
                                         y_lp=self._lp_out_stem(m[1], Bx, Hx, Wx, x.requires_grad, dx_channels)), True,
                         out_lp=self._lp_edge(first, 2, False))
        base = 4 + 3 * self.n_down
        twin = None
        for i in range(self.n_down):
# ... 128 lines not shown
```

mmhand_amd/ops.py:

```python
import ctypes as C
import os
import weakref

import torch

from . import lib as L


def _ptr(t):
    return None if t is None else C.c_void_p(t.data_ptr())


_raw_stream = getattr(torch._C, "_cuda_getCurrentRawStream", None)
_raw_device = getattr(torch._C, "_cuda_getDevice", None)


def _stream():
    if _raw_stream is not None and _raw_device is not None:
        return C.c_void_p(_raw_stream(_raw_device()))
    return C.c_void_p(torch.cuda.current_stream().cuda_stream)


def _chk(t, name="tensor"):
    if not (t.is_cuda and t.dtype == torch.float32 and t.is_contiguous()):
# ... 377 lines not shown
        L.call("mmh_wino_input_normact", _ptr(pro.x), B, H, W_, Cin, int(bool(reflect)), _ptr(V), _ptr(pro.scale),
               _ptr(pro.shift), pro.groups, int(pro.relu), float(pro.drop_p), _ptr(pro.drows), _stream())
    else:
        L.call("mmh_wino_input", _ptr(x), B, H, W_, Cin, 2 if fold else int(bool(reflect)), tile, dt, _ptr(V), _stream())
    if timed:
        e0.record()
    if levels16:
        assert tile == 2 and not bf16
        L.call("mmh_wino_gemm_levels16", _ptr(V), _ptr(U), _ptr(M), tiles, Cin, Cout, levels16, _stream())
    elif levels and not bf16:
        L.call("mmh_wino_gemm_levels", _ptr(V), _ptr(U), _ptr(M), tiles, Cin, Cout, P, levels, _stream())
    else:
        L.call("mmh_wino_gemm", _ptr(V), _ptr(U), _ptr(M), tiles, Cin, Cout, P, dt, _stream())
    if timed:
        e1.record()
    _count("mfma", 2.0 * P * tiles * Cin * Cout)
    stats = None
    if want_stats and FUSE_NORM_STATS and tile == 6 and not bf16 and act == L.ACT_NONE:
        stats = _empty((B, tiles // B, 3, Cout), x)
    L.call("mmh_wino_output", _ptr(M), _ptr(y), _ptr(bias), B, H, W_, Cout, act, tile, dt, _ptr(stats),
           int(bool(fold)), _stream())
    if timed:
        o1.record()
    if stats is not None:
        _park_stats(y, stats)
    return (y, V) if keep_V else y


def raw_conv_fprop_wino(x, w, bias, reflect, act=L.ACT_NONE, tile=4, keep_V=False, bf16=False, pro=None):
    if pro is None:
        _chk(x, "x")
    _chk(w, "w")
    return _wino_conv(x, wino_weights(w, tile, False, bf16), bias, w.shape[3], reflect, act, tile, time_it=True,
                      keep_V=keep_V, bf16=bf16, want_stats=True, pro=pro)


def raw_conv_dgrad_wino(dy, w, x_shape, reflect, tile=4, bf16=False):
    _chk(dy, "dy"); _chk(w, "w")
    B, H, W_, Cin = x_shape
    Cout = w.shape[3]
    if reflect and tile == 6 and not bf16 and _fold_ok(H, W_):
        return _wino_conv(dy, wino_weights(w, tile, True, bf16), None, Cin, False, L.ACT_NONE, tile, fold=True,
                          levels=WINO_DGRAD_LEVELS)
    dx = _wino_conv(dy, wino_weights(w, tile, True, bf16), None, Cin, False, L.ACT_NONE, tile, bf16=bf16, levels=WINO_DGRAD_LEVELS)
    if reflect:
        d = conv_desc(B, H, W_, Cin, Cout, 3, 1, 1, True)
        wb = w
        if bf16 and Cout % 64 == 0:
            d.dtype = _dt(bf16)
            wb = bf16_weights(w, bf16)[0]
        ws = _ws(L.load().mmh_conv2d_dgrad_border_ws_bytes(C.byref(d)), dy)
        L.call("mmh_conv2d_dgrad_border", C.byref(d), _ptr(dy), _ptr(wb), _ptr(dx), _ptr(ws), ws.numel() * 4, 3,
               0, _stream())
    return dx


def raw_conv_wgrad_wino(x, dy, reflect, tile=4, V=None, bf16=False, out=None):
    _chk(dy, "dy")
    B, H, W_, Cout = dy.shape
    P = (tile + 2) ** 2
    tiles = B * (-(-H // tile)) * (-(-W_ // tile))
    dt = _dt(bf16)
    wd = _wd(bf16)
    if V is None:
        _chk(x, "x")
        Cin = x.shape[3]
        V = torch.empty((P, tiles, Cin), dtype=wd, device=dy.device)
        L.call("mmh_wino_input", _ptr(x), B, H, W_, Cin, int(bool(reflect)), tile, dt, _ptr(V), _stream())
    else:
        Cin = V.shape[2]
        assert tuple(V.shape) == (P, tiles, Cin) and V.is_contiguous() and V.dtype == wd
    Yh = torch.empty((P, tiles, Cout), dtype=wd, device=dy.device)
    L.call("mmh_wino_dy", _ptr(dy), B, H, W_, Cout, tile, dt, _ptr(Yh), _stream())
    ws = _ws(L.load().mmh_wino_wgrad_gemm_ws_bytes(tiles, Cin, Cout, P), dy)
    dU = _empty((P, Cin, Cout), dy)
    L.call("mmh_wino_wgrad_gemm", _ptr(V), _ptr(Yh), tiles, Cin, Cout, P, dt, _ptr(ws), ws.numel() * 4, _ptr(dU),
           _stream())
    _count("mfma", 2.0 * P * tiles * Cin * Cout)
    dw = out if out is not None else _empty((3, 3, Cin, Cout), dy)
    L.call("mmh_wino_dw", _ptr(dU), Cin, Cout, tile, _ptr(dw), int(out is not None), _stream())
    return dw


def raw_conv_bwd_wino6(dy, w, x_shape, reflect, V, dw_out=None, nbd=None):
    _chk(w, "w")
    B, H, W_, Cin = x_shape
    Cout = w.shape[3]
    P, tile = 64, 6
    tiles = B * (-(-H // tile)) * (-(-W_ // tile))
    assert tuple(V.shape) == (P, tiles, Cin) and V.is_contiguous() and V.dtype == torch.float32
    fold = bool(reflect) and _fold_same_grid(H, W_)
    if nbd is not None:
        dy = nbd.g
        assert tuple(dy.shape) == (B, H, W_, Cout) and tuple(nbd.x.shape) == tuple(dy.shape)
        Vd = _empty((P, tiles, Cout), dy)
        Yh = _empty((P, tiles, Cout), dy)
        L.call("mmh_wino_input_dy_normbwd", _ptr(nbd.g), _ptr(nbd.x), B, H, W_, Cout, _ptr(Vd), _ptr(Yh), int(fold),
               _ptr(nbd.mean), _ptr(nbd.invstd), _ptr(nbd.gamma), _ptr(nbd.s1), _ptr(nbd.s2), float(nbd.count),
               _ptr(nbd.scale), _ptr(nbd.shift), _ptr(nbd.drows), nbd.groups, int(nbd.relu), float(nbd.drop_p),
               _stream())
    else:
        _chk(dy, "dy")
        Vd = _empty((P, tiles, Cout), dy)
        Yh = _empty((P, tiles, Cout), dy)
        L.call("mmh_wino_input_dy", _ptr(dy), B, H, W_, Cout, tile, L.F32, _ptr(Vd), _ptr(Yh), int(fold), _stream())
    M = _empty((P, tiles, Cin), dy)
    if WINO_DGRAD_LEVELS:
        L.call("mmh_wino_gemm_levels", _ptr(Vd), _ptr(wino_weights(w, tile, True)), _ptr(M), tiles, Cout, Cin, P, WINO_DGRAD_LEVELS,
               _stream())
    else:
        L.call("mmh_wino_gemm", _ptr(Vd), _ptr(wino_weights(w, tile, True)), _ptr(M), tiles, Cout, Cin, P, L.F32, _stream())
    _count("mfma", 2.0 * 2 * P * tiles * Cin * Cout)
    dx = _empty((B, H, W_, Cin), dy)
    L.call("mmh_wino_output", _ptr(M), _ptr(dx), None, B, H, W_, Cin, L.ACT_NONE, tile, L.F32, None, int(fold),
           _stream())
    if reflect and not fold:
        assert nbd is None, "the border GEMMs read dy: the caller materialises it (Conv2dFn.backward)"
        d = conv_desc(B, H, W_, Cin, Cout, 3, 1, 1, True)
        ws = _ws(L.load().mmh_conv2d_dgrad_border_ws_bytes(C.byref(d)), dy)
        L.call("mmh_conv2d_dgrad_border", C.byref(d), _ptr(dy), _ptr(w), _ptr(dx), _ptr(ws), ws.numel() * 4, 3,
               0, _stream())
    ws = _ws(L.load().mmh_wino_wgrad_gemm_ws_bytes(tiles, Cin, Cout, P), dy)
    dU = _empty((P, Cin, Cout), dy)
    L.call("mmh_wino_wgrad_gemm", _ptr(V), _ptr(Yh), tiles, Cin, Cout, P, L.F32, _ptr(ws), ws.numel() * 4, _ptr(dU),
           _stream())
    dw = dw_out if dw_out is not None else _empty((3, 3, Cin, Cout), dy)
    L.call("mmh_wino_dw", _ptr(dU), Cin, Cout, tile, _ptr(dw), int(dw_out is not None), _stream())
    return dx, dw


def raw_conv_fprop(x, w, bias, stride, pad, reflect, act=L.ACT_NONE, bf16=False, want_stats=False):
    _chk(x, "x"); _chk(w, "w")
    B, H, W_, Cin = x.shape
    k, _, wc, Cout = w.shape
    assert wc == Cin, f"weight Cin {wc} != x channels {Cin}"
    wt = _wino_tile(B, H, W_, Cin, Cout, k, stride, pad, bf16)
    if wt:
        return raw_conv_fprop_wino(x, w, bias, reflect, act, wt, bf16=bf16)
    if not bf16 and _wino2_fwd_ok(x, H, W_, Cin, Cout, k, stride, pad):
        return _wino_conv(x, wino_weights(w, 2), bias, Cout, reflect, act, 2, levels16=2)
    d = conv_desc(B, H, W_, Cin, Cout, k, stride, pad, reflect)
    y = _empty((B, d.Ho, d.Wo, Cout), x)
    if USE_THIN and k == 7 and stride == 1 and pad == 3 and Cout == 4 and Cin % 4 == 0:
        if bf16 and conv7_n4_ok(d, 0, bf16):
            return raw_conv7_n4(d, 0, lp16_twin(x, bf16), w, bias, y, act, bf16)
        L.call("mmh_conv7_thin_fprop", C.byref(d), _ptr(x), _ptr(w), _ptr(bias), _ptr(y), act, _stream())
        _count_desc("valu", d)
        return y
    if bf16 and lp16_v2_ok(Cin, Cout, k, stride, pad, 0):
        timed = fprop_timer is not None and fprop_timer.want(d)
        x16 = lp16_twin(x, bf16)
        if timed:
            e0, e1 = fprop_timer.bracket()
            e0.record()
        y = raw_conv3x3_lp16(x16, w, bias, reflect, act, bf16, 0)
        if timed:
            e1.record()
        return y
    if bf16 and lp16g_ok(d, 0, bf16):
        return raw_conv_lp16g(d, 0, lp16_twin(x, bf16), w, bias, act, bf16)
    if bf16 and lp16_flat_ok(d, bf16):
        timed = fprop_timer is not None and fprop_timer.want(d)
        if timed:
            e0, e1 = fprop_timer.bracket()
            e0.record()
        y = raw_conv_lp16_flat(d, x, w, bias, act, bf16)
        if timed:
            e1.record()
        return y
    if bf16:
        d.dtype = _dt(bf16)
        w = bf16_weights(w, bf16)[1]
    _count_desc("mfma", d)
    if (want_stats and FUSE_NORM_STATS and not bf16 and act == L.ACT_NONE and (d.Ho * d.Wo) % 128 == 0
            and not (fprop_timer is not None and fprop_timer.want(d))):
        chunks = L.load().mmh_conv2d_fprop_stats_chunks(C.byref(d))
        if chunks > 0:
            stats = _empty((B, chunks // B, 3, Cout), x)
            L.call("mmh_conv2d_fprop_stats", C.byref(d), _ptr(x), _ptr(w), _ptr(bias), _ptr(y), _ptr(stats), _stream())
            _park_stats(y, stats)
            return y
    if fprop_timer is not None and fprop_timer.want(d):
        e0, e1 = fprop_timer.bracket()
        e0.record()
        L.call("mmh_conv2d_fprop", C.byref(d), _ptr(x), _ptr(w), _ptr(bias), _ptr(y), act, _stream())
        e1.record()
        return y
    L.call("mmh_conv2d_fprop", C.byref(d), _ptr(x), _ptr(w), _ptr(bias), _ptr(y), act, _stream())
    return y


USE_CONV7_N4 = os.environ.get("MMH_CONV7_N4", "1") != "0"


def conv7_n4_ok(d, mode, lp):
    if not (USE_CONV7_N4 and lp):
        return False
    keep = d.dtype
    d.dtype = _dt(lp)
    ok = bool(L.load().mmh_conv7_n4_lp16_supported(C.byref(d), mode))
    d.dtype = keep
    return ok


# ... 520 lines not shown
        out = torch.empty(L.load().mmh_conv_stem16_weights_bytes_k(c8, ks) // 2, dtype=_wd(bf16), device=w.device)
        L.call("mmh_prep_weights_stem16_k", _ptr(w), cin, c8, ks, _dt(bf16), _ptr(out), _stream())
        ent = _cache_put(_stem16_cache, key, w, out)
    return ent


USE_STEM3 = os.environ.get("MMH_STEM3", "1") != "0"


def raw_conv_lp16_flat(d, x, w, bias, act, bf16, out16=False, x16p=None, want_stats=False):
    c8 = (d.Cin + 7) // 8 * 8
    if x16p is None:
        x16p = lp16_pad8(x, bf16)
    d.dtype = _dt(bf16)
    y = torch.empty((d.B, d.H, d.W, d.Cout), dtype=_wd(bf16) if out16 else torch.float32, device=x16p.device)
    if (USE_STEM_FPROP16 and (d.kh == 7 or (d.kh == 3 and USE_STEM3)) and w.shape[3] == 64
            and L.load().mmh_conv_stem16_supported(C.byref(d), c8)):
        chunks = (L.load().mmh_conv_stem16_stats_chunks(C.byref(d), c8)
                  if (want_stats and FUSE_NORM_STATS and FUSE_NORM_STATS_NARROW and out16 and act == L.ACT_NONE) else 0)
        if chunks > 0:
            stats = torch.empty((d.B, chunks, 3, d.Cout), dtype=torch.float32, device=x16p.device)
            L.call("mmh_conv_stem16_stats", C.byref(d), _ptr(x16p), c8, _ptr(stem16_weights(w, bf16)), _ptr(bias), _ptr(y),
                   _ptr(stats), _ptr(zero_page(x16p.device)), _stream())
            _park_stats(y, stats)
            _count_desc("mfma", d)
            return y
        L.call("mmh_conv_stem16", C.byref(d), _ptr(x16p), c8, _ptr(stem16_weights(w, bf16)), _ptr(bias), _ptr(y),
               int(out16), act, _ptr(zero_page(x16p.device)), _stream())
        _count_desc("mfma", d)
        return y
    L.call("mmh_conv_lp16_flat", C.byref(d), _ptr(x16p), c8, _ptr(flat8_weights(w, bf16)), _ptr(bias), _ptr(y),
           int(out16), act, _ptr(zero_page(x16p.device)), _stream())
    _count_desc("mfma", d)
    return y


def stem_lp16_ok(d, bf16, dx_channels):
    return (lp16_flat_ok(d, bf16) and d.kh == 7 and d.stride == 1 and d.pad == 3 and USE_THIN
            and 0 <= dx_channels <= 4 and d.Cout % 4 == 0)


def lp16_chain_ok(Cin, Cout, k, stride, pad, reflect=True, bf16=True):
    if not (USE_LP16_V2 and k == 3 and pad == 1):
        return False
    if (lp16_v2_ok(Cin, Cout, k, stride, pad, 0) and lp16_v2_ok(Cin, Cout, k, stride, pad, 1)
            and lp16_wgrad_ok(Cin, Cout, k, stride, pad)):
        return True
    d = conv_desc(1, 8, 8, Cin, Cout, k, stride, pad, reflect)
    fprop = lp16_v2_ok(Cin, Cout, k, stride, pad, 0) or lp16g_ok(d, 0, bf16)
    dgrad = lp16_v2_ok(Cin, Cout, k, stride, pad, 1) or (not reflect and lp16g_ok(d, 1, bf16))
    return fprop and dgrad and Cin % 4 == 0 and Cout % 4 == 0


def convT_lp16_ok(CinT, CoutT, bf16=True):
    d = conv_desc(1, 8, 8, CoutT, CinT, 3, 2, 1, False)
    return USE_LP16_V2 and lp16g_ok(d, 0, bf16) and lp16g_ok(d, 1, bf16)


def _tdt(t):
    return {torch.float32: L.F32, torch.bfloat16: L.BF16, torch.float16: L.FP16}[t.dtype]


_lp_grads = {}


def lp_grad_out(t16):
    p = lp_proxy(t16.shape, t16.device)
    _lp_grads[p.data_ptr()] = (p, t16)
    return p


def lp_grad_in(g, what):
    ent = _lp_grads.pop(g.data_ptr(), None) if g is not None else None
    if ent is None or tuple(ent[1].shape) != tuple(g.shape):
        raise RuntimeError(f"{what}: the gradient of a 16-bit edge did not arrive through the 16-bit channel "
                           "(an edge with more than one consumer, or a foreign backward node)")
    return ent[1]


def lp_grads_reset():
    _lp_grads.clear()
    _nb_defer.clear()
    _nbr_sites.clear()
    for k in [k for k, ent in _pack_twins.items() if not ent[3]]:
        del _pack_twins[k]


USE_NORM_FUSION = os.environ.get("MMH_FUSE_NORMACT", "1") != "0"


class NormDefer:
    __slots__ = ("x", "scale", "shift", "groups", "relu", "drop_p", "drows")

    def __init__(self, x, scale, shift, groups, relu, drop_p, drows):
        self.x, self.scale, self.shift, self.groups = x, scale, shift, groups
        self.relu, self.drop_p, self.drows = relu, drop_p, drows


class NormBwdDefer:
    __slots__ = ("g", "x", "mean", "invstd", "gamma", "s1", "s2", "count", "scale", "shift", "dbits", "drows", "groups",
                 "rows", "relu", "drop_p")


_nb_defer = {}


def norm_bwd_defer_out(ent):
    p = lp_proxy(ent.x.shape, ent.x.device)
    _nb_defer[p.data_ptr()] = (p, ent)
    return p


def norm_bwd_defer_in(g, what):
    ent = _nb_defer.pop(g.data_ptr(), None) if g is not None else None
    if ent is None or tuple(ent[1].x.shape) != tuple(g.shape):
        raise RuntimeError(f"{what}: expected the deferred gradient of a fused norm (NormBwdDefer) on this edge")
    return ent[1]


def raw_norm_bwd_apply_rc(e):
    dx = torch.empty_like(e.x)
    L.call("mmh_norm_bwd_apply_rc", _ptr(e.g), _ptr(e.x), _ptr(e.mean), _ptr(e.invstd), _ptr(e.gamma), _ptr(e.s1),
           _ptr(e.s2), _ptr(e.scale), _ptr(e.shift), _ptr(e.dbits), float(e.count), e.groups, e.rows, e.x.shape[3],
           int(e.relu), float(e.drop_p), _ptr(dx), _stream())
    return dx


def raw_dropout_bits(shape, drop_p, seed, mask, device, rows=False):
    n = 1
    for d in shape:
        n *= d
    bits = torch.empty((n // 8,), dtype=torch.uint8, device=device)
    if not rows:
        L.call("mmh_dropout_bits", n, float(drop_p), seed, _ptr(mask), _ptr(bits), _stream())
        return bits
    B, H, W_, Cc = shape
    drows = torch.empty((B * H, (W_ + 31) // 32, Cc), dtype=torch.int32, device=device)
    L.call("mmh_dropout_bits_both", B * H, W_, Cc, float(drop_p), seed, _ptr(mask), _ptr(bits), _ptr(drows), _stream())
    return bits, drows


def norm_fusion_ok(C):
    c8 = C // 8
    return USE_NORM_FUSION and C % 8 == 0 and 1 <= c8 <= 256 and (c8 & (c8 - 1)) == 0


ACCUM_PARAM_GRADS = False
EXACT_NULL_BIAS_GRAD = os.environ.get("MMH_NULL_BIAS_GRAD", "exact") != "compute"


def _grad_target(p):
    if ACCUM_PARAM_GRADS and p is not None and p.requires_grad and p.grad is not None and p.grad.is_contiguous() \
            and p.grad.dtype == torch.float32 and p.grad.shape == p.shape:
        return p.grad
    return None


def _dp_use(ctx_needs, w, bias):
    from . import dp
    if dp.tracking():
        if ctx_needs[1]:
            dp.param_use(w)
        if bias is not None and ctx_needs[2]:
            dp.param_use(bias)


def _dp_done(ctx_needs, w, bias, dw, db):
    from . import dp
    if dp.tracking():
        if ctx_needs[1] and dw is None:
            dp.param_done(w)
        if bias is not None and ctx_needs[2] and db is None:
            dp.param_done(bias)


DP_NO_COMM = os.environ.get("MMH_DP_NO_COMM") == "1"


def _finish_param_grad(g, target):
    return None if target is not None else g


def lp_proxy(shape, device):
    return torch.empty_strided(tuple(shape), (0,) * len(shape), dtype=torch.float32, device=device)
# ... 63 lines not shown
    _chk16(x, "x"); _chk16(dy, "dy")
    assert bf16 or (x.dtype == torch.float32 and dy.dtype == torch.float32)
    B, h, w_, CinT = x.shape
    CoutT = dy.shape[3]
    d = conv_desc(B, 2 * h, 2 * w_, CoutT, CinT, 3, 2, 1, False)
    if bf16:
        d.dtype = _dt(bf16)
    if bf16 and (x.dtype != torch.float32 or dy.dtype != torch.float32) and lp16_flat_wgrad_ok(d, CoutT, bf16):
        x = x if x.dtype != torch.float32 else lp16_twin(x, bf16)
        dy = dy if dy.dtype != torch.float32 else lp16_twin(dy, bf16)
        dd = conv_desc(B, 2 * h, 2 * w_, CoutT, CinT, 3, 2, 1, False)
        return raw_wgrad_lp16_flat(dd, dy, CoutT, x, bf16, out=out)
    if x.dtype != dy.dtype:
        x = x if x.dtype != torch.float32 else lp16_twin(x, bf16)
        dy = dy if dy.dtype != torch.float32 else lp16_twin(dy, bf16)
    nbytes = L.load().mmh_conv2d_wgrad_ws_bytes(C.byref(d))
    ws = _ws(nbytes, x)
    dw = out if out is not None else _empty((3, 3, CoutT, CinT), x)
    L.call("mmh_convT2d_wgrad", C.byref(d), _ptr(x), _ptr(dy), _ptr(dw), _ptr(ws),
           ws.numel() * 4, int(out is not None),
           (1 if x.dtype != torch.float32 else 0) | (2 if dy.dtype != torch.float32 else 0), _stream())
    _count_desc("mfma", d)
    return dw


def raw_colsum(x2d_rows, Ccols, x, out=None):
    ws = torch.empty(L.load().mmh_colsum_ws_bytes(x2d_rows, Ccols) // 4 + 4, dtype=torch.float32, device=x.device)
    acc = out is not None
    if out is None:
        out = torch.empty((Ccols,), dtype=torch.float32, device=x.device)
    L.call("mmh_colsum", _ptr(x), x2d_rows, Ccols, Ccols, _ptr(out), _ptr(ws), ws.numel() * 4, int(acc), _tdt(x),
           _stream())
    return out


def raw_act_bwd_lp16(g, y, act, lp):
    _chk(g, "g"); _chk(y, "y")
    out = torch.empty(g.shape, dtype=_wd(lp), device=g.device)
    L.call("mmh_act_bwd_lp16", _ptr(g), _ptr(y), g.numel(), act, _dt(lp), _ptr(out), _stream())
    return out


def raw_act_bwd(g, y, act):
    g = g.contiguous()
    dx = torch.empty_like(g)
    L.call("mmh_act_bwd", _ptr(g), _ptr(y), _ptr(dx), g.numel(), act, _stream())
    return dx


def _tok_add(dx, addend):
    if addend is None:
        return dx
    assert dx is not None and dx.dtype == torch.float32, "a parked residual gradient needs an fp32 input gradient to join"
    return dx.add_(addend)


class Conv2dFn(torch.autograd.Function):

    @staticmethod
    def forward(ctx, x, w, bias, stride, pad, reflect, act, bf16=False, dx_channels=0, x16=None, y_lp=False,
                null_bias_grad=False, pro=None, g_defer=False, res_tok=None, x_twin=None):
        ctx.set_materialize_grads(False)
        _dp_use(ctx.needs_input_grad, w, bias)
        ctx.res_tok = res_tok
        if res_tok is not None:
            assert x16 is None and pro is None, "a residual token belongs to an fp32 block input"
            res_tok.armed = bool(ctx.needs_input_grad[0])
            res_tok.taken = False
        ctx.g_defer = bool(g_defer)
        ctx.skip_db = bool(null_bias_grad and EXACT_NULL_BIAS_GRAD)
        ctx.bias_p = bias
        B, H, W_, Cin = x.shape
        ctx.dx_channels = dx_channels
        wt = _wino_tile(B, H, W_, Cin, w.shape[3], w.shape[0], stride, pad, bf16)
        ctx.cfg = (stride, pad, reflect, act, bias is not None, bf16)
        ctx.x_shape = tuple(x.shape)
        ctx.wino_V = 0
        ctx.lp16 = False
        ctx.x_lp = x16 is not None
        ctx.y_lp = bool(y_lp)
        k = w.shape[0]
        ctx.stem16 = ctx.head16 = False
        ctx.nbr = nbr_site_take(x16) if (x16 is not None and torch.is_tensor(x16)) else None
        if pro is not None:
            assert wt == 6 and not bf16 and x16 is None and not y_lp, "a deferred norm needs the fp32 F(6x6,3x3) path"
            if KEEP_WINOGRAD_INPUT and ctx.needs_input_grad[1]:
                y, V = raw_conv_fprop_wino(x, w, bias, reflect, act, wt, keep_V=True, pro=pro)
                ctx.wino_V = wt
                ctx.save_for_backward(V, w, y if act != L.ACT_NONE else None)
                return y
            assert not ctx.needs_input_grad[1], "a deferred norm in front of a trainable conv needs MMH_WINOGRAD_KEEP_INPUT=1"
            y = raw_conv_fprop_wino(x, w, bias, reflect, act, wt, pro=pro)
            ctx.save_for_backward(None, w, y if act != L.ACT_NONE else None)
            return y
        chain = bool(bf16) and lp16_chain_ok(Cin, w.shape[3], k, stride, pad, reflect, bf16)
        head16 = bool(bf16) and k == 7 and not y_lp and not dx_channels and pro is None \
            and head16_ok(B, H, W_, Cin, w.shape[3], k, stride, pad, reflect, bf16)
        if x16 is not None:
            assert (chain or head16) and x16.dtype == _wd(bf16) and tuple(x16.shape) == tuple(x.shape), \
                "a 16-bit input needs 16-bit kernels for all three passes"
        ctx.stem16 = False
        ctx.head16 = head16
        if head16:
            if x16 is None:
                x16 = lp16_twin(x, bf16)
            d = conv_desc(B, H, W_, Cin, w.shape[3], k, stride, pad, reflect)
            y = torch.empty((B, H, W_, w.shape[3]), dtype=torch.float32, device=x16.device)
            raw_conv7_n4(d, 0, x16, w, bias, y, act, bf16)
            ctx.save_for_backward(x16, w, y if act != L.ACT_NONE else None)
            return y
        if y_lp and not chain:
            d = conv_desc(B, H, W_, Cin, w.shape[3], k, stride, pad, reflect)
            assert bf16 and act == L.ACT_NONE and x16 is None and stem_lp16_ok(d, bf16, dx_channels), \
                "a 16-bit output needs 16-bit kernels for all passes and no activation"
            x16p = lp16_pad8(x, bf16)
            y = raw_conv_lp16_flat(d, None, w, bias, act, bf16, out16=True, x16p=x16p, want_stats=bool(null_bias_grad))
            ctx.stem16 = True
            ctx.save_for_backward(x16p, w, None)
            ctx.mark_non_differentiable(y)
            return lp_proxy(y.shape, y.device), y
        if y_lp:
            assert act == L.ACT_NONE, "a 16-bit output needs no activation"
        v2 = bool(bf16) and lp16_v2_ok(Cin, w.shape[3], k, stride, pad, 0)
        if v2 or chain:
            if x16 is None:
                if x_twin is not None and v2 and USE_LP16_CAT_TWIN:
                    assert x_twin.dtype == _wd(bf16) and tuple(x_twin.shape) == tuple(x.shape)
                    x16 = x_twin
                else:
                    x16 = lp16_twin(x, bf16)
            d = conv_desc(B, H, W_, Cin, w.shape[3], k, stride, pad, reflect)
            timed = fprop_timer is not None and fprop_timer.want(d)
            if timed:
                e0, e1 = fprop_timer.bracket()
                e0.record()
            if v2:
                y = raw_conv3x3_lp16(x16, w, bias, reflect, act, bf16, 0, out16=bool(y_lp),
                                     want_stats=bool(null_bias_grad and y_lp))
            else:
                y = raw_conv_lp16g(d, 0, x16, w, bias, act, bf16, out16=bool(y_lp), want_stats=bool(null_bias_grad and y_lp))
            if timed:
                e1.record()
            ctx.lp16 = chain or lp16_wgrad_ok(Cin, w.shape[3], k, stride, pad)
            ctx.save_for_backward(x16 if ctx.lp16 else x, w, y if act != L.ACT_NONE else None)
            if y_lp:
                ctx.mark_non_differentiable(y)
                return lp_proxy(y.shape, y.device), y
            return y
        if wt and KEEP_WINOGRAD_INPUT and ctx.needs_input_grad[1]:
            y, V = raw_conv_fprop_wino(x, w, bias, reflect, act, wt, keep_V=True, bf16=bf16)
            ctx.wino_V = wt
            ctx.save_for_backward(V, w, y if act != L.ACT_NONE else None)
            return y
        y = raw_conv_fprop(x, w, bias, stride, pad, reflect, act, bf16, want_stats=bool(null_bias_grad))
        ctx.save_for_backward(x, w, y if act != L.ACT_NONE else None)
        return y

    @staticmethod
    def backward(ctx, g, _g16=None):
        out = Conv2dFn._backward(ctx, g, _g16)
        _dp_done(ctx.needs_input_grad, ctx.saved_tensors[1], ctx.bias_p, out[1], out[2])
        return out

    @staticmethod
    def _backward(ctx, g, _g16=None):
        addend = ctx.res_tok.take() if ctx.res_tok is not None else None
        x, w, y = ctx.saved_tensors
        stride, pad, reflect, act, has_bias, bf16 = ctx.cfg
        dx = dw = db = None
        if g is None:
            return (addend,) + (None,) * 15
        wt_ = _grad_target(w) if ctx.needs_input_grad[1] else None
        bt_ = _grad_target(ctx.bias_p) if (has_bias and ctx.needs_input_grad[2]) else None
        want_db = has_bias and ctx.needs_input_grad[2] and not ctx.skip_db
        if has_bias and ctx.needs_input_grad[2] and ctx.skip_db and (ctx.bias_p.grad is None or not ACCUM_PARAM_GRADS):
            db = torch.zeros_like(ctx.bias_p)
        if (act != L.ACT_NONE and bf16 and ctx.needs_input_grad[0] and not ctx.needs_input_grad[1] and not want_db
                and not ctx.g_defer and not ctx.y_lp and not ctx.x_lp and not ctx.dx_channels
                and _dgrad_takes_dy16(*ctx.x_shape, w.shape[3], w.shape[0], stride, pad, reflect, bf16)):
            g16 = raw_act_bwd_lp16(g.contiguous(), y, act, bf16)
            dx = raw_conv_dgrad(None, w, ctx.x_shape, stride, pad, reflect, bf16, 0, dy16=g16)
            return _tok_add(dx, addend), dw, db, None, None, None, None, None, None, None, None, None, None, None, None, None
        if ctx.head16:
            g = g.contiguous()
            if act != L.ACT_NONE:
                g = raw_act_bwd(g, y, act)
            if ctx.needs_input_grad[0]:
                dx = raw_conv_dgrad(g, w, ctx.x_shape, stride, pad, reflect, bf16, 0, out16=ctx.x_lp)
                if ctx.x_lp:
                    dx = lp_grad_out(dx)
            if ctx.needs_input_grad[1]:
                dw = _finish_param_grad(raw_head_wgrad16(x, g, bf16, out=wt_), wt_)
            if want_db:
                db = _finish_param_grad(raw_colsum(g.numel() // g.shape[3], g.shape[3], g, out=bt_), bt_)
            return _tok_add(dx, addend), dw, db, None, None, None, None, None, None, None, None, None, None, None, None, None
        if ctx.stem16:
            g16 = lp_grad_in(g, "Conv2dFn (stem)")
            if ctx.needs_input_grad[0]:
                dx = raw_conv_dgrad_thin(g16, w, ctx.x_shape, reflect)
            if ctx.needs_input_grad[1]:
                Bx, Hx, Wx, Cx = ctx.x_shape
                dd = conv_desc(Bx, Hx, Wx, Cx, w.shape[3], w.shape[0], stride, pad, reflect)
                if stem_wgrad16_ok(dd, x.shape[3], bf16) and g16.is_contiguous():
                    dw = _finish_param_grad(raw_wgrad_stem_lp16(dd, x, g16, bf16, out=wt_), wt_)
                elif lp16_flat_wgrad_ok(dd, x.shape[3], bf16):
                    dw = _finish_param_grad(raw_wgrad_lp16_flat(dd, x, x.shape[3], g16, bf16, out=wt_), wt_)
                else:
                    dw = _finish_param_grad(raw_conv_wgrad_lp16_gen1(x, g16, Cx, w.shape[0], stride, pad, reflect, bf16,
                                                                     out=wt_), wt_)
            if want_db:
                db = _finish_param_grad(raw_colsum(g16.numel() // g16.shape[3], g16.shape[3], g16, out=bt_), bt_)
            return _tok_add(dx, addend), dw, db, None, None, None, None, None, None, None, None, None, None, None, None, None
        if ctx.y_lp:
            g16 = lp_grad_in(g, "Conv2dFn")
            if ctx.needs_input_grad[0]:
                fuse = addend is not None and not ctx.x_lp and not ctx.dx_channels
                dx = raw_conv_dgrad(None, w, ctx.x_shape, stride, pad, reflect, bf16, ctx.dx_channels, dy16=g16,
                                    out16=ctx.x_lp, addend=addend if fuse else None,
                                    nbr=ctx.nbr if (ctx.x_lp and not ctx.dx_channels) else None)
                if fuse:
                    addend = None
                if ctx.x_lp:
                    dx = lp_grad_out(dx)
            if ctx.needs_input_grad[1]:
                dw = _finish_param_grad(raw_conv_wgrad(x, g16, w.shape[0], stride, pad, reflect, bf16, out=wt_), wt_)
            if want_db:
                db = _finish_param_grad(raw_colsum(g16.numel() // g16.shape[3], g16.shape[3], g16, out=bt_), bt_)
            return _tok_add(dx, addend), dw, db, None, None, None, None, None, None, None, None, None, None, None, None, None
        fused_bwd = (FUSE_WINO6_BWD and ctx.wino_V == 6 and not bf16 and ctx.needs_input_grad[0]
                     and ctx.needs_input_grad[1]
                     and _wino_tile(*ctx.x_shape, w.shape[3], 3, stride, pad, bf16, "dgrad") == 6)
        nbd = None
        if ctx.g_defer:
            nbd = norm_bwd_defer_in(g, "Conv2dFn")
            Hx, Wx = ctx.x_shape[1], ctx.x_shape[2]
            if not (fused_bwd and act == L.ACT_NONE and not want_db and (not reflect or _fold_same_grid(Hx, Wx))):
                g = raw_norm_bwd_apply_rc(nbd)
                nbd = None
        if nbd is None:
            g = g.contiguous()
            if act != L.ACT_NONE:
                g = raw_act_bwd(g, y, act)
        if fused_bwd:
            dx, dw = raw_conv_bwd_wino6(g, w, ctx.x_shape, reflect, x, dw_out=wt_, nbd=nbd)
            dw = _finish_param_grad(dw, wt_)
            if want_db:
                db = _finish_param_grad(raw_colsum(g.numel() // g.shape[3], g.shape[3], g, out=bt_), bt_)
            return _tok_add(dx, addend), dw, db, None, None, None, None, None, None, None, None, None, None, None, None, None
        if ctx.lp16:
            g16 = lp16_twin(g, bf16)
            if ctx.needs_input_grad[0]:
                dx = raw_conv_dgrad(g, w, ctx.x_shape, stride, pad, reflect, bf16, ctx.dx_channels, dy16=g16,
                                    out16=ctx.x_lp)
                if ctx.x_lp:
                    dx = lp_grad_out(dx)
            if ctx.needs_input_grad[1]:
                dw = _finish_param_grad(raw_conv_wgrad(x, g16, w.shape[0], stride, pad, reflect, bf16, out=wt_), wt_)
            if want_db:
                db = _finish_param_grad(raw_colsum(g.numel() // g.shape[3], g.shape[3], g, out=bt_), bt_)
            return _tok_add(dx, addend), dw, db, None, None, None, None, None, None, None, None, None, None, None, None, None
        if (not WINOGRAD_FPROP and FUSE_WINO6_BWD and not bf16 and not ctx.wino_V and not ctx.dx_channels
                and ctx.needs_input_grad[0] and ctx.needs_input_grad[1] and x is not None and x.dtype == torch.float32
                and _wino_tile(*ctx.x_shape, w.shape[3], w.shape[0], stride, pad, bf16, "dgrad") == 6
                and _wino_tile(*ctx.x_shape, w.shape[3], w.shape[0], stride, pad, bf16, "wgrad") == 6):
            Bx, Hx, Wx, Cx = ctx.x_shape
            V = _empty((64, Bx * (-(-Hx // 6)) * (-(-Wx // 6)), Cx), x)
            L.call("mmh_wino_input", _ptr(x), Bx, Hx, Wx, Cx, int(bool(reflect)), 6, L.F32, _ptr(V), _stream())
            dx, dw = raw_conv_bwd_wino6(g, w, ctx.x_shape, reflect, V, dw_out=wt_)
            dw = _finish_param_grad(dw, wt_)
            if want_db:
                db = _finish_param_grad(raw_colsum(g.numel() // g.shape[3], g.shape[3], g, out=bt_), bt_)
            return _tok_add(dx, addend), dw, db, None, None, None, None, None, None, None, None, None, None, None, None, None
        if ctx.needs_input_grad[0]:
            dx = raw_conv_dgrad(g, w, ctx.x_shape, stride, pad, reflect, bf16, ctx.dx_channels)
        if ctx.needs_input_grad[1]:
            if ctx.wino_V:
                dw = _finish_param_grad(raw_conv_wgrad_wino(None, g, reflect, ctx.wino_V, V=x, bf16=bf16, out=wt_), wt_)
            else:
                dw = _finish_param_grad(raw_conv_wgrad(x, g, w.shape[0], stride, pad, reflect, bf16, out=wt_), wt_)
        if want_db:
            db = _finish_param_grad(raw_colsum(g.numel() // g.shape[3], g.shape[3], g, out=bt_), bt_)
        return _tok_add(dx, addend), dw, db, None, None, None, None, None, None, None, None, None, None, None, None, None


class ConvT2dFn(torch.autograd.Function):

    @staticmethod
    def forward(ctx, x, w, bias, bf16=False, x16=None, y_lp=False, null_bias_grad=False):
        ctx.set_materialize_grads(False)
        _dp_use(ctx.needs_input_grad, w, bias)
        ctx.skip_db = bool(null_bias_grad and EXACT_NULL_BIAS_GRAD)
        ctx.bias_p = bias
        ctx.has_bias = bias is not None
        ctx.bf16 = bf16
        ctx.x_lp = x16 is not None
        ctx.y_lp = bool(y_lp)
        ctx.x_shape = tuple(x.shape)
        chain = bool(bf16) and convT_lp16_ok(x.shape[3], w.shape[2], bf16)
        if x16 is not None or y_lp:
            assert chain, "16-bit edges of a ConvTranspose2d need 16-bit kernels for all three passes"
        if chain:
            if x16 is None:
                x16 = lp16_twin(x, bf16)
            y = raw_convT_fprop(x16, w, bias, L.ACT_NONE, bf16, out16=bool(y_lp))
            ctx.lp16 = True
            ctx.save_for_backward(x16, w)
            if y_lp:
                ctx.mark_non_differentiable(y)
                return lp_proxy(y.shape, y.device), y
            return y
        ctx.lp16 = False
        y = raw_convT_fprop(x, w, bias, L.ACT_NONE, bf16)
        ctx.save_for_backward(x, w)
        return y

    @staticmethod
    def backward(ctx, g, _g16=None):
        out = ConvT2dFn._backward(ctx, g, _g16)
        _dp_done(ctx.needs_input_grad, ctx.saved_tensors[1], ctx.bias_p, out[1], out[2])
        return out

    @staticmethod
    def _backward(ctx, g, _g16=None):
        x, w = ctx.saved_tensors
        dx = dw = db = None
        if g is None:
            return (None,) * 7
        wt_ = _grad_target(w) if ctx.needs_input_grad[1] else None
        bt_ = _grad_target(ctx.bias_p) if (ctx.has_bias and ctx.needs_input_grad[2]) else None
        if ctx.has_bias and ctx.needs_input_grad[2] and ctx.skip_db and (ctx.bias_p.grad is None or not ACCUM_PARAM_GRADS):
            db = torch.zeros_like(ctx.bias_p)
# ... 223 lines not shown
def _sync_bwd_sums_inplace(packed, pairs, group):
    import torch.distributed as dist
    if DP_NO_COMM:
        return list(pairs), list(pairs)
    collective_counter["all_reduce"] = collective_counter.get("all_reduce", 0) + 1
    if len(pairs) > 1:
        collective_counter["packed_sites"] = collective_counter.get("packed_sites", 0) + len(pairs)
    local = packed.clone()
    dist.all_reduce(packed, group=group)
    loc, off = [], 0
    for s1, s2 in pairs:
        n = s1.numel()
        loc.append((local[off:off + n].view_as(s1), local[off + n:off + 2 * n].view_as(s2)))
        off += 2 * n
    return loc, list(pairs)


class _SiteCtx:

    def __init__(self):
        self.saved_tensors, self.nondiff = (), []

    def save_for_backward(self, *t):
        self.saved_tensors = t

    def mark_non_differentiable(self, *t):
        self.nondiff += list(t)


def _norm_fwd_local(ctx, x, gamma, beta, mode, relu, drop_p, out_lp, x16, stat_out=None):
    ctx.in_lp = x16 is not None
    ctx.out_lp = bool(out_lp)
    if x16 is not None:
        assert tuple(x16.shape) == tuple(x.shape) and x16.is_contiguous()
        x = x16
    else:
        _chk(x, "x")
    if drop_p > 0 and not relu:
        raise RuntimeError("NormActFn: dropout without a preceding ReLU is not supported")
    B = x.shape[0]
    groups = B if mode == "instance" else 1
    fast = raw_norm_stats_finalize_pending(x, groups) if (mode == "instance" and gamma is None and beta is None) else None
    if fast is not None:
        return x, groups, fast, None, None, fast[4]
    mean, m2, rows = raw_norm_stats(x, groups, out=stat_out)
    return x, groups, None, mean, m2, rows


USE_NORM_TWIN = os.environ.get("MMH_NORM_TWIN", "1") != "0"


def norm_twin_ok(C):
    c8 = C // 8
    return USE_NORM_TWIN and USE_LP16_CAT_TWIN and C % 8 == 0 and 1 <= c8 <= 256 and (c8 & (c8 - 1)) == 0


def _norm_fwd_finish(ctx, st, synced, gamma, beta, residual, running_mean, running_var, relu, drop_p, seed, mask,
                     sync_group, out_lp, x16, defer, want_twin=0):
    x, groups, fast, mean, m2, rows = st
    if fast is not None:
        mean, scale, shift, invstd, rows = fast
        count = rows
    else:
        count = rows
        if synced is not None:
            mean, m2, count = synced
        if isinstance(mean, _GatheredStats):
            mean, m2, scale, shift, invstd = mean.finalize(gamma, beta, running_mean, running_var)
        else:
            scale, shift, invstd = raw_norm_finalize(mean, m2, count, gamma, beta, running_mean, running_var)
    ctx.defer = int(defer)
    if defer == 3:
        assert (x16 is None and not out_lp and not relu and drop_p == 0 and x.dtype == torch.float32
                and norm_fusion_ok(x.shape[3]))
        out = raw_scale_shift_act(x, scale, shift, residual, False, 0.0, 0, None)
        ctx.cfg = (groups, rows, count, False, 0.0, sync_group, residual is not None)
        ctx.save_for_backward(x, None, mean, invstd, gamma, scale, shift, None)
        return (out,)
    if defer:
        assert x16 is None and not out_lp and residual is None and x.dtype == torch.float32 and norm_fusion_ok(x.shape[3])
        dbits, drows = raw_dropout_bits(x.shape, drop_p, seed, mask, x.device, rows=True) if drop_p > 0 else (None, None)
        ctx.cfg = (groups, rows, count, bool(relu), float(drop_p), sync_group, False)
        ctx.save_for_backward(x, dbits, mean, invstd, gamma, scale, shift, drows)
        ctx.mark_non_differentiable(scale, shift)
        if drows is not None:
            ctx.mark_non_differentiable(drows)
        return lp_proxy(x.shape, x.device), scale, shift, drows
    masked = bool(relu or drop_p > 0)
    twin_lp = want_twin if (want_twin and not out_lp and norm_twin_ok(x.shape[3])) else 0
    r = raw_scale_shift_act(x, scale, shift, residual, relu, drop_p, seed, mask, keep_bits=masked, out_lp=out_lp,
                            twin_lp=twin_lp)
    r = r if isinstance(r, tuple) else (r,)
    out, kb, twin = r[0], (r[1] if masked else None), (r[-1] if twin_lp else None)
    ctx.cfg = (groups, rows, count, bool(relu), float(drop_p), sync_group,
               residual is not None)
    ctx.save_for_backward(x, kb, mean, invstd, gamma)
    ctx.nbr_site = None
    if (USE_NBR and out_lp and masked and residual is None and x.dtype != torch.float32 and x.shape[3] >= NBR_MIN_C
            and x.shape[3] % 256 == 0):
        ctx.nbr_site = NormBwdSite(x, kb, mean, invstd, groups, float(drop_p))
        nbr_site_put(out, ctx.nbr_site)
    if want_twin and not out_lp:
        if twin is not None:
            ctx.mark_non_differentiable(twin)
        return out, twin
    if out_lp:
        if residual is not None:
            raise RuntimeError("NormActFn: a 16-bit output together with a residual is not supported")
        ctx.mark_non_differentiable(out)
        return lp_proxy(x.shape, x.device), out
    return (out,)


USE_NORM_BWD_PLANE = os.environ.get("MMH_NORM_BWD_PLANE", "0") == "1"


def _norm_bwd_local(ctx, g, sums_out=None):
    groups, rows, count, relu, drop_p, sync_group, has_res = ctx.cfg
    ctx.fused_dx = None
    if ctx.defer:
        x, dbits, mean, invstd, gamma, scale, shift, drows = ctx.saved_tensors
        g = g.contiguous()
        Cc = x.shape[3]
        ws = _ws(L.load().mmh_norm_bwd_ws_bytes(groups, rows, Cc), x)
        s1, s2 = sums_out if sums_out is not None else (_empty((groups, Cc), x), _empty((groups, Cc), x))
        L.call("mmh_norm_bwd_reduce_rc", _ptr(g), _ptr(x), _ptr(mean), _ptr(invstd), _ptr(scale), _ptr(shift),
               _ptr(dbits), groups, rows, Cc, int(relu), drop_p, _ptr(s1), _ptr(s2), _ptr(ws), ws.numel() * 4, _stream())
        return g, s1, s2
    x, out, mean, invstd, gamma = ctx.saved_tensors
    if has_res and relu:
        raise RuntimeError("NormActFn: residual together with ReLU is not on the reference path")
    g = lp_grad_in(g, "NormActFn") if ctx.out_lp else g.contiguous()
    Cc = x.shape[3]
    masked = 2 if (relu or drop_p > 0) else 0
    site = getattr(ctx, "nbr_site", None)
    if site is not None and site.g is g and site.s1 is not None:
        s1, s2 = site.s1, site.s2
        site.g = site.s1 = site.s2 = None
        if sums_out is not None:
            sums_out[0].copy_(s1.view_as(sums_out[0]))
            sums_out[1].copy_(s2.view_as(sums_out[1]))
            s1, s2 = sums_out
        return g, s1, s2
    s1, s2 = sums_out if sums_out is not None else (_empty((groups, Cc), x), _empty((groups, Cc), x))
    if (USE_NORM_BWD_PLANE and sync_group is None and x.dtype != torch.float32 and g.dtype in (torch.float32, x.dtype)
            and L.load().mmh_norm_bwd_fused_supported(groups, rows, Cc, masked, _tdt(g), _tdt(x))):
        dx = torch.empty_like(x)
        L.call("mmh_norm_bwd_fused", _ptr(g), _ptr(out), _ptr(x), _ptr(mean), _ptr(invstd), _ptr(gamma), float(count),
               groups, rows, Cc, masked, drop_p, _ptr(s1), _ptr(s2), _ptr(dx), _tdt(g), _tdt(x), _tdt(dx), _stream())
        ctx.fused_dx = dx
        return g, s1, s2
    ws = _ws(L.load().mmh_norm_bwd_ws_bytes(groups, rows, Cc), x)
    L.call("mmh_norm_bwd_reduce", _ptr(g), _ptr(out), _ptr(x), _ptr(mean), _ptr(invstd), groups,
           rows, Cc, masked, drop_p, _ptr(s1), _ptr(s2), _ptr(ws), ws.numel() * 4, _tdt(g), _tdt(x), _stream())
    return g, s1, s2


def _norm_bwd_finish(ctx, g, s1l, s2l, s1, s2):
    groups, rows, count, relu, drop_p, sync_group, has_res = ctx.cfg
    gamma = ctx.saved_tensors[4]
    dgamma = dbeta = None
    if gamma is not None:
        own = (s1l is not s1 and s2l is not s2) or not ctx.defer
        dgamma = s2l.sum(0) if groups > 1 else (s2l.reshape(-1) if own else s2l.reshape(-1).clone())
        dbeta = s1l.sum(0) if groups > 1 else (s1l.reshape(-1) if own else s1l.reshape(-1).clone())
    if ctx.defer:
        x, dbits, mean, invstd, gamma, scale, shift, drows = ctx.saved_tensors
        e = NormBwdDefer()
        e.g, e.x, e.mean, e.invstd, e.gamma, e.s1, e.s2, e.count = g, x, mean, invstd, gamma, s1, s2, count
        e.scale, e.shift, e.dbits, e.drows = scale, shift, dbits, drows
        e.groups, e.rows, e.relu, e.drop_p = groups, rows, relu, drop_p
        dx = norm_bwd_defer_out(e) if ctx.defer >= 2 else raw_norm_bwd_apply_rc(e)
        return dx, dgamma, dbeta, (g if has_res else None)
    x, out, mean, invstd, gamma = ctx.saved_tensors
    Cc = x.shape[3]
    masked = 2 if (relu or drop_p > 0) else 0
    dx = getattr(ctx, "fused_dx", None)
    ctx.fused_dx = None
    if dx is None:
        dx = torch.empty_like(x)
        L.call("mmh_norm_bwd_apply", _ptr(g), _ptr(out), _ptr(x), _ptr(mean), _ptr(invstd),
               _ptr(gamma), _ptr(s1), _ptr(s2), float(count), groups, rows, Cc, masked, drop_p,
               _ptr(dx), _tdt(g), _tdt(x), _tdt(dx), _stream())
    dres = g if has_res else None
    if ctx.in_lp:
        dx = lp_grad_out(dx)
    return dx, dgamma, dbeta, dres


class NormActFn(torch.autograd.Function):

    @staticmethod
    def forward(ctx, x, gamma, beta, residual, running_mean, running_var, mode, relu, drop_p,
                seed, mask, sync_group, out_lp=0, x16=None, defer=0, res_tok=None, want_twin=0):
        ctx.set_materialize_grads(False)
        ctx.res_tok = res_tok if residual is not None else None
        st = _norm_fwd_local(ctx, x, gamma, beta, mode, relu, drop_p, out_lp, x16)
        synced = None
        if mode == "batch" and sync_group is not None and st[2] is None:
            synced = _sync_stats(st[3], st[4], st[5], sync_group)
        outs = _norm_fwd_finish(ctx, st, synced, gamma, beta, residual, running_mean, running_var, relu, drop_p, seed,
                                mask, sync_group, out_lp, x16, defer, want_twin if not defer else 0)
        if want_twin and not defer and not out_lp and outs[1] is None:
            return outs[0], None
        return outs[0] if len(outs) == 1 else outs

# ... 615 lines not shown
```

Baseline: 120.8 images/s.

## Fuse norm-backward sums and residual add into Winograd dgrad output transform

Adds a Winograd F(6x6,3x3) output-transform kernel that can fold the residual-gradient add into the dgrad output write, and can optionally compute the per-tile partial sums needed for the deferred instance-norm backward reduction. This drops a separate elementwise add pass and, when enabled, the separate norm-backward reduce kernel that would re-read g and x. Residual tokens are now enabled on the fp32 path too, so the add fusion takes effect by default. The norm-sums fusion stays behind an environment flag that defaults off. It also brings a scalar per-channel-thread kernel with double-precision accumulation and a partial-sums buffer, which may be slower than the existing vectorised output kernel.

```diff
diff --git a/include/mmhand_hip.h b/include/mmhand_hip.h
--- a/include/mmhand_hip.h
+++ b/include/mmhand_hip.h
@@ -256,6 +256,12 @@
                               const void* scale, const void* shift, const void* drows, int groups,
                               int relu, float drop_p, mmh_stream_t s);
 
+int mmh_wino_output_nbsums_supported(int B, int H, int W, int C, int groups);
+int mmh_wino_output_nbsums(const void* M, void* g, const void* addend, int B, int H, int W, int C, const void* y,
+                           const void* mean, const void* invstd, const void* scale, const void* shift,
+                           const void* drows, int groups, int relu, float drop_p, void* part, void* s1, void* s2,
+                           mmh_stream_t s);
+
 int mmh_act_bwd(const void* g, const void* y, void* dx, int64_t n, int act,
                 mmh_stream_t s);
 int mmh_act_bwd_lp16(const void* g, const void* y, int64_t n, int act, int dtype, void* out16,
diff --git a/mmhand_amd/csrc/common.h b/mmhand_amd/csrc/common.h
--- a/mmhand_amd/csrc/common.h
+++ b/mmhand_amd/csrc/common.h
@@ -127,6 +127,9 @@
 int wino6_output(const float* M, float* y, const float* bias, int B, int H, int W, int C, int act, float* stats,
                  int fold, hipStream_t st);
 int wino6_dy(const float* dy, float* Yh, int B, int H, int W, int C, hipStream_t st);
+int wino6_output_nbsums(const float* M, float* g, const float* addend, int B, int H, int W, int C, const float* y,
+                        const float* mean, const float* invstd, const float* scale, const float* shift,
+                        const uint32_t* drows, int groups, int relu, float drop_p, float* part, hipStream_t st);
 int wino6_input_normact(const float* x, float* V, int B, int H, int W, int C, int reflect, int xcd,
                         const float* scale, const float* shift, int groups, int relu, float drop_p,
                         const uint32_t* drows, hipStream_t st);
diff --git a/mmhand_amd/csrc/conv_igemm.hip b/mmhand_amd/csrc/conv_igemm.hip
--- a/mmhand_amd/csrc/conv_igemm.hip
+++ b/mmhand_amd/csrc/conv_igemm.hip
@@ -2744,6 +2744,8 @@
 
 int g_wino_bn256 = 0;
 int g_wino_xcd = 1;
+int g_wino_nbsums = 1;
+int g_wino_dgrad_add = 1;
 int g_wino_gemm_v2 = 1;
 int g_wino_bf16_bk = 64;
 int g_wino_bf16_occ = 3;
@@ -2953,6 +2955,8 @@
     if (!strcmp(key, "wino_wgrad_occ")) { g_wino_wgrad_occ = value; return 0; }
     if (!strcmp(key, "wino_gemm_v2")) { g_wino_gemm_v2 = value; return 0; }
     if (!strcmp(key, "wino_xcd")) { g_wino_xcd = value; return 0; }
+    if (!strcmp(key, "wino_nbsums")) { g_wino_nbsums = value; return 0; }
+    if (!strcmp(key, "wino_dgrad_add")) { g_wino_dgrad_add = value; return 0; }
     if (!strcmp(key, "dgrad_s2_multi")) { g_dgrad_s2_multi = value; return 0; }
     if (!strcmp(key, "wino6_vec")) { mmh::g_wino6_vec = value; return 0; }
     if (!strcmp(key, "lp16_shape")) { mmh::g_lp16_shape = value; return 0; }
@@ -3241,6 +3245,35 @@
                                static_cast<float*>(y), static_cast<const float*>(bias), B, H, W, C / 4, act);
     }
     return mmh::check_launch("wino_output_kernel");
+}
+
+int mmh_wino_output_nbsums_supported(int B, int H, int W, int C, int groups) {
+    if (B <= 0 || C <= 0 || C % 8 || !wino_fold_ok(H, W) || (long long)B * H * W * C >= (1ll << 31)) return 0;
+    return ((g_wino_nbsums && (groups == 1 || groups == B)) ? 1 : 0) | (g_wino_dgrad_add ? 2 : 0);
+}
+
+int mmh_wino_output_nbsums(const void* M, void* g, const void* addend, int B, int H, int W, int C, const void* y,
+                           const void* mean, const void* invstd, const void* scale, const void* shift,
+                           const void* drows, int groups, int relu, float drop_p, void* part, void* s1, void* s2,
+                           mmh_stream_t s) {
+    MMH_REQUIRE(M && g && B > 0 && C > 0 && C % 8 == 0 && wino_fold_ok(H, W) && (long long)B * H * W * C < (1ll << 31),
+                "mmh_wino_output_nbsums: bad arguments (fp32 fold: (H+1) %% 6 >= 2, C %% 8 == 0, numel < 2^31)");
+    if (y)
+        MMH_REQUIRE(mean && invstd && scale && shift && part && s1 && s2 && (groups == 1 || groups == B) && drop_p >= 0.f &&
+                        drop_p < 1.f && (drop_p == 0.f) == (drows == nullptr),
+                    "mmh_wino_output_nbsums: bad norm arguments (groups 1 | B, dropout rows iff p > 0)");
+    else
+        MMH_REQUIRE(addend && !drows, "mmh_wino_output_nbsums: neither a norm nor an addend (mmh_wino_output does that)");
+    if (int rc = mmh::wino6_output_nbsums(static_cast<const float*>(M), static_cast<float*>(g),
+                                          static_cast<const float*>(addend), B, H, W, C, static_cast<const float*>(y),
+                                          static_cast<const float*>(mean), static_cast<const float*>(invstd),
+                                          static_cast<const float*>(scale), static_cast<const float*>(shift),
+                                          static_cast<const uint32_t*>(drows), groups, relu, y ? drop_p : 0.f,
+                                          static_cast<float*>(part), mmh::as_stream(s)))
+        return rc;
+    if (!y) return 0;
+    const int tpi = ((H + 7) / 6) * ((W + 7) / 6);
+    return mmh_norm_bwd_sums_final(part, groups, C, groups == 1 ? B * tpi : tpi, s1, s2, s);
 }
 
 static int wino_wgrad_splits(int Cin, int Cout, long long tiles, int nbatch) {
diff --git a/mmhand_amd/csrc/wino6.hip b/mmhand_amd/csrc/wino6.hip
--- a/mmhand_amd/csrc/wino6.hip
+++ b/mmhand_amd/csrc/wino6.hip
@@ -368,6 +368,120 @@
         float* o = stats + ((long long)(b * (TH * TW) + ty * TW + tx) * 3) * C2 + c;
         o[0] = n; o[C2] = mean; o[2 * C2] = m2;
     }
+}
+
+struct NormSums {
+    const float* addend;
+    const float* y;
+    const float* mean;
+    const float* invstd;
+    float* part;
+    int relu;
+    NormPro np;
+};
+
+template <bool DROP, bool ADD, bool SUMS>
+__global__ void __launch_bounds__(256) wino6_output_nbsums_kernel(const float* __restrict__ M, float* __restrict__ g, int B,
+                                                                  int H, int W, int C, const NormSums ns) {
+    const int TH = (H + 7) / 6, TW = (W + 7) / 6;
+    const long long tiles = (long long)B * TH * TW;
+    const long long i = (long long)blockIdx.x * blockDim.x + threadIdx.x;
+    if (i >= tiles * C) return;
+    const int c = (int)(i % C);
+    const long long tile = i / C;
+    const int tx = (int)(tile % TW), ty = (int)((tile / TW) % TH), b = (int)(tile / ((long long)TW * TH));
+    bool okh[6], okw[6];
+    unsigned rowi[6], ro[6], co[6];
+    int ww[6];
+#pragma unroll
+    for (int r = 0; r < 6; ++r) {
+        const int ph = 6 * ty + r, pw = 6 * tx + r;
+        okh[r] = ph >= 1 && ph <= H; okw[r] = pw >= 1 && pw <= W;
+        ww[r] = okw[r] ? pw - 1 : 0;
+        rowi[r] = (unsigned)(b * H + (okh[r] ? ph - 1 : 0));
+        ro[r] = rowi[r] * (unsigned)W * (unsigned)C;
+        co[r] = (unsigned)ww[r] * (unsigned)C + (unsigned)c;
+    }
+    float av[ADD ? 6 : 1][6], yv[SUMS ? 6 : 1][6];
+    uint32_t lo[DROP ? 6 : 1], hi[DROP ? 6 : 1];
+    int wq0 = 6 * tx - 1;
+    wq0 = (wq0 < 0 ? 0 : wq0) >> 5;
+    const int wq1 = wq0 + 1 < ns.np.nW32 ? wq0 + 1 : wq0;
+#pragma unroll
+    for (int r = 0; r < 6; ++r) {
+#pragma unroll
+        for (int q = 0; q < 6; ++q) {
+            if (ADD) av[r][q] = ns.addend[ro[r] + co[q]];
+            if (SUMS) yv[r][q] = ns.y[ro[r] + co[q]];
+        }
+        if (DROP) {
+            lo[r] = ns.np.drows[(rowi[r] * (unsigned)ns.np.nW32 + (unsigned)wq0) * (unsigned)C + (unsigned)c];
+            hi[r] = ns.np.drows[(rowi[r] * (unsigned)ns.np.nW32 + (unsigned)wq1) * (unsigned)C + (unsigned)c];
+        }
+    }
+    const long long plane = tiles * C;
+    const float* in = M + tile * C + c;
+    float s6[6][8], colv[8], o6[6];
+#pragma unroll
+    for (int q = 0; q < 8; ++q) {
+#pragma unroll
+        for (int r = 0; r < 8; ++r) colv[r] = in[(long long)(r * 8 + q) * plane];
+        w6_at(colv, o6);
+#pragma unroll
+        for (int r = 0; r < 6; ++r) s6[r][q] = o6[r];
+    }
+    float vals[6][6];
+#pragma unroll
+    for (int r = 0; r < 6; ++r) {
+        w6_at(s6[r], o6);
+#pragma unroll
+        for (int q = 0; q < 6; ++q) vals[r][q] = o6[q];
+    }
+    const int rb = H + 1 - 6 * ty, cb = W + 1 - 6 * tx;
+#pragma unroll
+    for (int q = 0; q < 6; ++q) {
+        if (ty == 0) vals[2][q] = vals[2][q] + vals[0][q];
+#pragma unroll
+        for (int r = 2; r < 6; ++r)
+            if (r == rb) vals[r - 2][q] = vals[r - 2][q] + vals[r][q];
+    }
+#pragma unroll
+    for (int r = 0; r < 6; ++r) {
+        if (tx == 0) vals[r][2] = vals[r][2] + vals[r][0];
+#pragma unroll
+        for (int q = 2; q < 6; ++q)
+            if (q == cb) vals[r][q - 2] = vals[r][q - 2] + vals[r][q];
+    }
+    if (ADD) {
+#pragma unroll
+        for (int r = 0; r < 6; ++r)
+#pragma unroll
+            for (int q = 0; q < 6; ++q) vals[r][q] = vals[r][q] + av[r][q];
+    }
+#pragma unroll
+    for (int r = 0; r < 6; ++r)
+#pragma unroll
+        for (int q = 0; q < 6; ++q)
+            if (okh[r] && okw[q]) g[ro[r] + co[q]] = vals[r][q];
+    if (!SUMS) return;
+    const int gi = (ns.np.per_image ? b : 0) * C + c;
+    const float sc = ns.np.scale[gi], sf = ns.np.shift[gi], mu = ns.mean[gi], is = ns.invstd[gi];
+    double p1 = 0., p2 = 0.;
+#pragma unroll
+    for (int r = 0; r < 6; ++r)
+#pragma unroll
+        for (int q = 0; q < 6; ++q) {
+            bool keep = okh[r] && okw[q] && (!ns.relu || __builtin_fmaf(yv[r][q], sc, sf) > 0.f);
+            if (DROP) {
+                const uint32_t wsel = (ww[q] >> 5) == wq0 ? lo[r] : hi[r];
+                keep = keep && ((wsel >> (ww[q] & 31)) & 1u);
+            }
+            const float gg = keep ? vals[r][q] * ns.np.dsc : 0.f;
+            p1 += (double)gg;
+            p2 = __builtin_fma((double)gg, (double)((yv[r][q] - mu) * is), p2);
+        }
+    float* o = ns.part + (tile * 2) * C + c;
+    o[0] = (float)p1; o[C] = (float)p2;
 }
 
 template <typename T>
@@ -621,6 +735,22 @@
     return check_launch("wino6_output_kernel");
 }
 
+int wino6_output_nbsums(const float* M, float* g, const float* addend, int B, int H, int W, int C, const float* y,
+                        const float* mean, const float* invstd, const float* scale, const float* shift,
+                        const uint32_t* drows, int groups, int relu, float drop_p, float* part, hipStream_t st) {
+    const long long tiles = (long long)B * ((H + 7) / 6) * ((W + 7) / 6);
+    const unsigned nblk = (unsigned)((tiles * C + 255) / 256);
+    NormSums ns{addend, y, mean, invstd, part, relu,
+                NormPro{scale, shift, drows, (W + 31) / 32, groups == 1 ? 0 : 1, 0.f, 1.f / (1.f - drop_p)}};
+#define MMH_NBSUMS_(D, A, S) \
+    hipLaunchKernelGGL((wino6_output_nbsums_kernel<D, A, S>), dim3(nblk), dim3(256), 0, st, M, g, B, H, W, C, ns)
+    if (!y) MMH_NBSUMS_(false, true, false);
+    else if (drows) { if (addend) MMH_NBSUMS_(true, true, true); else MMH_NBSUMS_(true, false, true); }
+    else { if (addend) MMH_NBSUMS_(false, true, true); else MMH_NBSUMS_(false, false, true); }
+#undef MMH_NBSUMS_
+    return check_launch("wino6_output_nbsums_kernel");
+}
+
 int wino6_dy(const float* dy, float* Yh, int B, int H, int W, int C, hipStream_t st) {
     const long long tiles = (long long)B * ((H + 5) / 6) * ((W + 5) / 6);
     if (g_wino6_vec & 4)
diff --git a/mmhand_amd/lib.py b/mmhand_amd/lib.py
--- a/mmhand_amd/lib.py
+++ b/mmhand_amd/lib.py
@@ -148,6 +148,9 @@
     "mmh_wino_input_normact": (_i, [_vp, _i, _i, _i, _i, _i, _vp, _vp, _vp, _i, _i, _f, _vp, _vp]),
     "mmh_wino_input_dy_normbwd": (_i, [_vp, _vp, _i, _i, _i, _i, _vp, _vp, _i, _vp, _vp, _vp, _vp, _vp, _d, _vp, _vp,
                                        _vp, _i, _i, _f, _vp]),
+    "mmh_wino_output_nbsums_supported": (_i, [_i, _i, _i, _i, _i]),
+    "mmh_wino_output_nbsums": (_i, [_vp, _vp, _vp, _i, _i, _i, _i, _vp, _vp, _vp, _vp, _vp, _vp, _i, _i, _f, _vp, _vp, _vp,
+                                    _vp]),
     "mmh_act_bwd": (_i, [_vp, _vp, _vp, _i64, _i, _vp]),
     "mmh_act_bwd_lp16": (_i, [_vp, _vp, _i64, _i, _i, _vp, _vp]),
     "mmh_act_bwd_lp16_io": (_i, [_vp, _i, _vp, _i, _i64, _i, _i, _vp, _vp]),
diff --git a/mmhand_amd/networks.py b/mmhand_amd/networks.py
--- a/mmhand_amd/networks.py
+++ b/mmhand_amd/networks.py
@@ -324,11 +324,11 @@
             assert self.training and x16 is None and not out_lp and not relu and not drop
             if self.norm == "instance":
                 return ops.NormActFn.apply(x, None, None, residual, None, None, "instance", False, 0.0, 0, None, None,
-                                           0, None, 3)
+                                           0, None, 3, res_tok)
             np_ = bag[idx]
             np_.count_batch()
             return ops.NormActFn.apply(x, np_.weight, np_.bias, residual, np_.running_mean, np_.running_var, "batch",
-                                       False, 0.0, 0, None, self.sync_group, 0, None, 3)
+                                       False, 0.0, 0, None, self.sync_group, 0, None, 3, res_tok)
         if defer:
             assert self.training and x16 is None and residual is None and not out_lp
             if self.norm == "instance":
@@ -380,9 +380,10 @@
                 and ops._wino_tile(B, H, W, Cin, Cout, 3, 1, 1, False) == 6
                 and ops._wino_tile(B, H, W, Cin, Cout, 3, 1, 1, False, "dgrad") == 6)
 
-    def _res_token(self, x):
-        return ops.ResidualToken() if (ops.USE_RESIDUAL_TOKENS and self.bf16 and self.training and torch.is_tensor(x)
-                                       and x.requires_grad) else None
+    def _res_token(self, x, c1):
+        if not (ops.USE_RESIDUAL_TOKENS and self.training and torch.is_tensor(x) and x.requires_grad):
+            return None
+        return ops.ResidualToken() if (self.bf16 or ops.wino_dgrad_add_ok(x.shape, c1.weight.shape[3])) else None
 
     def _twin_for(self, cp):
         if not (self.bf16 and self.training and cp is not None and cp.k == 3 and not cp.transposed):
@@ -392,7 +393,7 @@
 
     def two_conv_block(self, blk, x, site, last_norm, residual=None, res_tok=None, x_twin=None, want_twin=0):
         if residual is not None and residual is x and last_norm:
-            res_tok = self._res_token(x)
+            res_tok = self._res_token(x, blk[1])
         i2 = 6 if self.use_dropout else 5
         fuse = self._norm_fusion(blk[1], blk[i2], x)
         fuse_last = 3 if (last_norm and last_norm != "gate" and torch.is_tensor(x) and self._norm_bwd_fusion(blk[i2], x)) else 0
@@ -544,7 +545,7 @@
                     [dict(net=self, blk=blk[f"conv_block_stream{s}"], x=x, site=p + str(s), last_norm=s == 1)
                      for s, x in zip((1, 2, 3), (x1, x2, x3))])
             else:
-                tok = self._res_token(x1)
+                tok = self._res_token(x1, blk["conv_block_stream1"][1])
                 i2 = 6 if self.use_dropout else 5
                 gate_norm = bool(self.norm == "instance" and self.training and self.bf16 and torch.is_tensor(x1)
                                  and self._lp_out(blk["conv_block_stream1"][i2])
diff --git a/mmhand_amd/ops.py b/mmhand_amd/ops.py
--- a/mmhand_amd/ops.py
+++ b/mmhand_amd/ops.py
@@ -483,7 +483,7 @@
     return dw
 
 
-def raw_conv_bwd_wino6(dy, w, x_shape, reflect, V, dw_out=None, nbd=None):
+def raw_conv_bwd_wino6(dy, w, x_shape, reflect, V, dw_out=None, nbd=None, site=None, addend=None):
     _chk(w, "w")
     B, H, W_, Cin = x_shape
     Cout = w.shape[3]
@@ -513,14 +513,29 @@
         L.call("mmh_wino_gemm", _ptr(Vd), _ptr(wino_weights(w, tile, True)), _ptr(M), tiles, Cout, Cin, P, L.F32, _stream())
     _count("mfma", 2.0 * 2 * P * tiles * Cin * Cout)
     dx = _empty((B, H, W_, Cin), dy)
-    L.call("mmh_wino_output", _ptr(M), _ptr(dx), None, B, H, W_, Cin, L.ACT_NONE, tile, L.F32, None, int(fold),
-           _stream())
+    if (site is not None and addend is None and fold and USE_WINO_NBSUMS and tuple(site.x.shape) == (B, H, W_, Cin)
+            and wino_nbsums_caps(B, H, W_, Cin, site.groups) & 1):
+        part = _empty((tiles, 2, Cin), dy)
+        site.s1, site.s2 = _empty((site.groups, Cin), dy), _empty((site.groups, Cin), dy)
+        L.call("mmh_wino_output_nbsums", _ptr(M), _ptr(dx), None, B, H, W_, Cin, _ptr(site.x), _ptr(site.mean),
+               _ptr(site.invstd), _ptr(site.scale), _ptr(site.shift), _ptr(site.drows), site.groups, int(site.relu),
+               site.drop_p, _ptr(part), _ptr(site.s1), _ptr(site.s2), _stream())
+        site.g = dx
+    elif (addend is not None and fold and USE_WINO_DGRAD_ADD and tuple(addend.shape) == (B, H, W_, Cin)
+          and addend.dtype == torch.float32 and addend.is_contiguous() and wino_nbsums_caps(B, H, W_, Cin, B) & 2):
+        L.call("mmh_wino_output_nbsums", _ptr(M), _ptr(dx), _ptr(addend), B, H, W_, Cin, None, None, None, None, None, None,
+               B, 0, 0.0, None, None, None, _stream())
+        addend = None
+    else:
+        L.call("mmh_wino_output", _ptr(M), _ptr(dx), None, B, H, W_, Cin, L.ACT_NONE, tile, L.F32, None, int(fold),
+               _stream())
     if reflect and not fold:
         assert nbd is None, "the border GEMMs read dy: the caller materialises it (Conv2dFn.backward)"
         d = conv_desc(B, H, W_, Cin, Cout, 3, 1, 1, True)
         ws = _ws(L.load().mmh_conv2d_dgrad_border_ws_bytes(C.byref(d)), dy)
         L.call("mmh_conv2d_dgrad_border", C.byref(d), _ptr(dy), _ptr(w), _ptr(dx), _ptr(ws), ws.numel() * 4, 3,
                0, _stream())
+    dx = _tok_add(dx, addend)
     ws = _ws(L.load().mmh_wino_wgrad_gemm_ws_bytes(tiles, Cin, Cout, P), dy)
     dU = _empty((P, Cin, Cout), dy)
     L.call("mmh_wino_wgrad_gemm", _ptr(V), _ptr(Yh), tiles, Cin, Cout, P, L.F32, _ptr(ws), ws.numel() * 4, _ptr(dU),
@@ -1207,6 +1222,7 @@
     _lp_grads.clear()
     _nb_defer.clear()
     _nbr_sites.clear()
+    _wino_norm_sites.clear()
     for k in [k for k, ent in _pack_twins.items() if not ent[3]]:
         del _pack_twins[k]
 
@@ -1225,6 +1241,47 @@
 class NormBwdDefer:
     __slots__ = ("g", "x", "mean", "invstd", "gamma", "s1", "s2", "count", "scale", "shift", "dbits", "drows", "groups",
                  "rows", "relu", "drop_p")
+
+
+USE_WINO_NBSUMS = os.environ.get("MMH_WINO_NBSUMS", "0") == "1"
+WINO_NBSUMS_MIN_C = int(os.environ.get("MMH_WINO_NBSUMS_MIN_C", "256"))
+
+
+USE_WINO_DGRAD_ADD = os.environ.get("MMH_WINO_DGRAD_ADD", "1") != "0"
+
+
+def wino_dgrad_add_ok(x_shape, Cout):
+    B, H, W_, Cin = x_shape
+    return bool(USE_WINO_DGRAD_ADD and USE_RESIDUAL_TOKENS and FUSE_WINO6_BWD and KEEP_WINOGRAD_INPUT and _fold_same_grid(H, W_)
+                and _wino_tile(B, H, W_, Cin, Cout, 3, 1, 1, False) == 6
+                and _wino_tile(B, H, W_, Cin, Cout, 3, 1, 1, False, "dgrad") == 6 and wino_nbsums_caps(B, H, W_, Cin, B) & 2)
+
+
+class WinoNormSite:
+    __slots__ = ("x", "mean", "invstd", "scale", "shift", "drows", "groups", "relu", "drop_p", "g", "s1", "s2")
+
+    def __init__(self, x, mean, invstd, scale, shift, drows, groups, relu, drop_p):
+        self.x, self.mean, self.invstd, self.scale, self.shift, self.drows = x, mean, invstd, scale, shift, drows
+        self.groups, self.relu, self.drop_p = groups, bool(relu), float(drop_p)
+        self.g = self.s1 = self.s2 = None
+
+
+_wino_norm_sites = {}
+
+
+def wino_norm_site_put(x, site):
+    while len(_wino_norm_sites) >= 8:
+        _wino_norm_sites.pop(next(iter(_wino_norm_sites)))
+    _wino_norm_sites[x.data_ptr()] = site
+
+
+def wino_norm_site_take(x):
+    site = _wino_norm_sites.pop(x.data_ptr(), None)
+    return site if (site is not None and site.x.data_ptr() == x.data_ptr() and tuple(site.x.shape) == tuple(x.shape)) else None
+
+
+def wino_nbsums_caps(B, H, W_, C_, groups):
+    return L.load().mmh_wino_output_nbsums_supported(B, H, W_, C_, groups)
 
 
 _nb_defer = {}
@@ -1454,8 +1511,10 @@
         k = w.shape[0]
         ctx.stem16 = ctx.head16 = False
         ctx.nbr = nbr_site_take(x16) if (x16 is not None and torch.is_tensor(x16)) else None
+        ctx.wino_site = None
         if pro is not None:
             assert wt == 6 and not bf16 and x16 is None and not y_lp, "a deferred norm needs the fp32 F(6x6,3x3) path"
+            ctx.wino_site = wino_norm_site_take(pro.x) if ctx.needs_input_grad[0] else None
             if KEEP_WINOGRAD_INPUT and ctx.needs_input_grad[1]:
                 y, V = raw_conv_fprop_wino(x, w, bias, reflect, act, wt, keep_V=True, pro=pro)
                 ctx.wino_V = wt
@@ -1614,11 +1673,12 @@
             if act != L.ACT_NONE:
                 g = raw_act_bwd(g, y, act)
         if fused_bwd:
-            dx, dw = raw_conv_bwd_wino6(g, w, ctx.x_shape, reflect, x, dw_out=wt_, nbd=nbd)
+            dx, dw = raw_conv_bwd_wino6(g, w, ctx.x_shape, reflect, x, dw_out=wt_, nbd=nbd,
+                                        site=ctx.wino_site, addend=addend)
             dw = _finish_param_grad(dw, wt_)
             if want_db:
                 db = _finish_param_grad(raw_colsum(g.numel() // g.shape[3], g.shape[3], g, out=bt_), bt_)
-            return _tok_add(dx, addend), dw, db, None, None, None, None, None, None, None, None, None, None, None, None, None
+            return dx, dw, db, None, None, None, None, None, None, None, None, None, None, None, None, None
         if ctx.lp16:
             g16 = lp16_twin(g, bf16)
             if ctx.needs_input_grad[0]:
@@ -2008,6 +2068,11 @@
         dbits, drows = raw_dropout_bits(x.shape, drop_p, seed, mask, x.device, rows=True) if drop_p > 0 else (None, None)
         ctx.cfg = (groups, rows, count, bool(relu), float(drop_p), sync_group, False)
         ctx.save_for_backward(x, dbits, mean, invstd, gamma, scale, shift, drows)
+        ctx.wino_site = None
+        if (USE_WINO_NBSUMS and sync_group is None and x.shape[3] >= WINO_NBSUMS_MIN_C
+                and wino_nbsums_caps(*x.shape, groups) & 1):
+            ctx.wino_site = WinoNormSite(x, mean, invstd, scale, shift, drows, groups, relu, drop_p)
+            wino_norm_site_put(x, ctx.wino_site)
         ctx.mark_non_differentiable(scale, shift)
         if drows is not None:
             ctx.mark_non_differentiable(drows)
@@ -2048,6 +2113,12 @@
         x, dbits, mean, invstd, gamma, scale, shift, drows = ctx.saved_tensors
         g = g.contiguous()
         Cc = x.shape[3]
+        site = getattr(ctx, "wino_site", None)
+        if site is not None:
+            sg, s1, s2 = site.g, site.s1, site.s2
+            site.g = site.s1 = site.s2 = None
+            if sg is g and s1 is not None and sums_out is None:
+                return g, s1, s2
         ws = _ws(L.load().mmh_norm_bwd_ws_bytes(groups, rows, Cc), x)
         s1, s2 = sums_out if sums_out is not None else (_empty((groups, Cc), x), _empty((groups, Cc), x))
         L.call("mmh_norm_bwd_reduce_rc", _ptr(g), _ptr(x), _ptr(mean), _ptr(invstd), _ptr(scale), _ptr(shift),
```

Result: no change. 121.2 images/s (median of 6 runs) (+0.3%).
